# nogueira04/RaCFormer

Measured on AMD Instinct MI355X. Metric: samples/sec (6-cam 704x256, 900 queries, f8), higher is better.
Workload: dtype f32

## Files before the change

### include/racformer_hip.h

```cpp
#ifndef RACFORMER_HIP_H
#define RACFORMER_HIP_H

#include <stdint.h>

#ifdef __cplusplus
extern "C" {
#endif

#define RAC_ABI_VERSION 8
#define RAC_MAX_LEVELS 8
#define RAC_MAX_POINTS 128

enum { RAC_F32 = 0, RAC_BF16 = 1, RAC_I16 = 2  };

enum {
    RAC_E_ARG = -1,
    RAC_E_UNSUPPORTED = -2,
};

enum {
    RAC_OUT_SQCP = 0,
    RAC_OUT_BQGTPC = 1
};

int rac_abi_version(void);
const char *rac_last_error(void);

int rac_msmv_fwd(const void *const *feats, const int32_t *hw, int L, const float *loc,
                 const float *w, float *out, int S, int N, int Q, int P, int C, int dtype,
                 int out_layout, int T, int G, void *stream);

int rac_msda_fwd(const void *value, const int64_t *shapes, const int64_t *starts, const float *loc,
                 const float *attn, float *out, int bs, int keys, int heads, int dim, int Q, int L,
                 int P, int dtype, void *stream);

int rac_regroup_fwd(const float *in, void *out, int B, int T, int N, int G, int C, int H, int W,
                    int out_dtype, void *stream);

int rac_regroup_multi_fwd(int L, const float *const *ins, void *const *outs, const int32_t *hw, int B, int T, int N, int G,
                          int C, int out_dtype, void *stream);

int rac_box_prep_fwd(const float *query_bbox, float *table, int num_boxes, const float *pc_range, void *stream);

int rac_sampling4d_fwd(const void *const *feats, const int32_t *hw, int L, const float *query_bbox,
                       const float *box_table, const float *offsets, const float *ray_logits, const float *scale_logits,
                       const float *time_diff, const float *lidar2img, float *out, float *loc_out,
                       float *w_out, const unsigned char *view_in, int ld_off, int ld_ray, int ld_scale, int B, int T, int N,
                       int G, int Q,
                       int NP, int D, int C, const float *pc_range, const float *depth_base, float d_region,
                       float image_h, float image_w, float eps, int dtype, int compact, void *stream);

int rac_bev_sampling_fwd(const void *value, const float *query_bbox, const float *box_table, const float *offsets,
                         const float *ray_logits, const float *scale_logits, const float *queue_logits,
                         const float *time_diff, float *out, float *loc_out, int ld_off, int ld_ray,
                         int ld_scale, int ld_queue, int B, int T, int Q, int heads, int NP, int D, int H, int W,
                         int dim, const float *pc_range, const float *depth_base, float d_region, int dtype,
                         void *stream);

int rac_bev_sampling_multi_fwd(int nstreams, const void *const *values, const float *const *offsets,
                               const float *const *ray_logits, const float *const *scale_logits,
                               const float *const *queue_logits, float *const *outs, const float *query_bbox,
                               const float *box_table, const float *time_diff, int ld_off, int ld_ray, int ld_scale,
                               int ld_queue, int B, int T, int Q, int heads, int NP, int D, int H, int W, int dim,
                               const float *pc_range, const float *depth_base, float d_region, int dtype, void *stream);

int rac_quant_i16_fwd(const float *values, void *q, float *scale, int64_t blocks, void *stream);

int rac_bev_sampling_multi_q16_fwd(int nstreams, const void *const *values, const float *const *value_scales,
                                   const float *const *offsets, const float *const *ray_logits,
                                   const float *const *scale_logits, const float *const *queue_logits, float *const *outs,
                                   const float *query_bbox, const float *box_table, const float *time_diff, int ld_off,
                                   int ld_ray, int ld_scale, int ld_queue, int B, int T, int Q, int heads, int NP, int D,
                                   int H, int W, int dim, const float *pc_range, const float *depth_base, float d_region,
                                   void *stream);

int rac_sasa_fwd(const float *qkv, const float *tau, const float *query_bbox, const float *box_table, float *out,
                 int ld_qkv, int ld_tau, int B, int Q, int heads, int dim, const float *pc_range, void *stream);

enum {
    RAC_SPLIT_KCAT = 0,
    RAC_SPLIT_LINES = 1
};

int rac_add_ln_fwd(const float *a, int num_partials, int64_t partial_stride, int ld_a, float a_scale, const float *residual,
                   const float *bias, const float *gamma, const float *beta, const float *post_residual,
                   float *out, int ld_out, int rows, int dim, float eps, int relu, void *split_out,
                   float split_scale, int split_pad, int split_layout, void *stream);

int rac_head_finish_fwd(float *cls, int64_t n_cls, const float *xy, float *box, int64_t rows, int code_size,
                        const float *pc_range, void *stream);

int rac_pe_head_fwd(const float *x, int ld_x, const float *weight, const float *bias, const float *gamma,
                    const float *beta, float *out, int rows, int dim, float eps, void *stream);

int rac_refine_fwd(const float *proposal, const float *delta, const float *time_diff_safe, float *bbox_pred,
                   float *bbox_xy, int B, int Q, int T, float num_ray, void *stream);

int rac_layer_boundary_fwd(const float *proposal, const float *delta, const float *time_diff_safe, float *bbox_pred,
                           float *bbox_xy, float *box_table, const float *pc_range, const float *pe_weight,
                           const float *pe_bias, const float *pe_gamma, const float *pe_beta, float *pe_out, int B, int Q,
                           int T, int dim, float num_ray, float eps, void *stream);

enum {
    RAC_MIX_F32 = 0,
    RAC_MIX_F16X3 = 1
};

int rac_mixing_fwd(const float *x, const float *params, float param_scale, float *out, void *out_split,
                   float split_scale, int ld_params, int num_query, int groups, int in_points, int channels, int out_points,
                   float eps, int mfma_mode, void *stream);

int rac_mixing_sampled_fwd(const void *const *feats, const int32_t *hw, int L, const float *query_bbox, const float *box_table,
                           const float *offsets, const float *ray_logits, const float *scale_logits, const float *time_diff,
                           const float *lidar2img, float *loc_out, float *w_out, const unsigned char *view_in, int ld_off,
                           int ld_ray, int ld_scale, int B, int T, int N, int G, int Q, int NP, int D, int C,
                           const float *pc_range, const float *depth_base, float d_region, float image_h, float image_w,
                           float eps_proj, int dtype, const float *params, float param_scale, float *out, void *out_split,
                           float split_scale, int ld_params, int out_points, float eps_ln, void *stream);

int rac_gemm_split_pack_fwd(const float *weight, void *image, int N, int K, float scale, void *stream);

int rac_outproj_fwd(const void *z_image, const void *w_image, float *partials, int M, int N, int K, int slices, void *stream);

int rac_generator_fwd(const void *x_image, const void *w_image, const float *bias, float alpha, float *out, int64_t ld_out, int M,
                      int N, int K, void *stream);

int rac_value_proj_fwd(const float *x, const void *w_image, float w_alpha, const float *add, const float *bias, float *out,
                       int frames, int channels, int HW, int features, void *stream);
int rac_value_proj_q16_fwd(const float *x, const void *w_image, float w_alpha, const float *add, const float *bias, void *q,
                           float *scale, int frames, int channels, int HW, int features, void *stream);

int rac_absmax_fwd(const float *const *srcs, const int64_t *counts, int num, float floor_value, float *amax_out,
                   void *stream);
int rac_conv_pack_fwd(const float *src, const float *amax, void *xs, int N, int C, int H, int W, int c_total,
                      int c_offset, void *stream);
int rac_conv_pack_bias_fwd(const float *src, const float *bias, const float *amax, void *xs, int N, int C, int H, int W,
                           int c_total, int c_offset, int frames_per_group, int live_per_group, void *stream);
int rac_conv3x3_fwd(const void *xs, const void *ws, const float *bias, const float *pixel_bias, const float *amax,
                    float w_alpha, float *out, int N, int H, int W, int Cin, int Cout, void *stream);
int rac_conv3x3_q16_fwd(const void *xs, const void *ws, const float *bias, const float *pixel_bias, const float *amax,
                        float w_alpha, void *q, float *scale, int N, int H, int W, int Cin, int Cout, void *stream);

int rac_fpn_conv_fwd(const void *xs, const void *ws, const float *bias, const float *amax, float w_alpha, float *out,
                     int num_images, int H, int W, int Cin, int num_cams, void *stream);

int rac_gru_gate_fwd(const float *gates, const float *h_prev, int64_t h_prev_bstride, float *h_out, int64_t h_out_bstride,
                     const float *bias_map, float *h_out2, int64_t h_out2_bstride, int B, int C, int HW, void *stream);
int rac_upsample2x_fwd(const float *src, float *dst, int64_t planes, int h, int w, void *stream);

#define RAC_ROWGEMM_MAX_BATCH 3
typedef struct {
    const float *a;
    int64_t partial_stride;
    const float *bias0, *residual, *gamma, *beta, *post;
    float *x_out;
    void *split_out;
    int ld_a, num_partials, ld_res, ld_post, ld_xout, relu, split_pad, split_layout;
    float a_scale, eps, split_scale;
} rac_rowseg;
typedef struct {
    rac_rowseg seg[3];
    const float *w, *b;
    float *out;
    int num_seg, N, ld_out, relu_from;
} rac_rowgemm;
int rac_rowgemm_fwd(const rac_rowgemm *descs, int num, int rows, void *stream);

int rac_conv3x3s2_fwd(const void *xs, const void *ws, const float *bias, const float *amax, float w_alpha, float *out,
                      int out_channels_total, int N, int H, int W, int Cin, int Cin_image, int Cout, void *stream);

int rac_decode_fwd(const float *cls_scores, const float *bbox_preds, float *out, int num_query, int num_classes,
                   int max_num, const float *post_center_range, float score_threshold, int use_threshold, void *stream);

int rac_msmv_bwd(const float *grad_out, const void *const *feats, const int32_t *hw, int L, const float *loc,
                 const float *w, void *const *grad_feats, float *grad_loc, float *grad_w, int S, int N, int Q,
                 int P, int C, void *stream);
int rac_msda_bwd(const float *grad_out, const float *value, const int64_t *shapes, const int64_t *starts,
                 const float *loc, const float *attn, float *grad_value, float *grad_loc, float *grad_attn,
                 int bs, int keys, int heads, int dim, int Q, int L, int P, void *stream);

int rac_bev_pool_v2_fwd(const float *depth, const float *feat, float *out, const int32_t *ranks_depth,
                        const int32_t *ranks_feat, const int32_t *ranks_bev, const int32_t *interval_lengths,
                        const int32_t *interval_starts, int c, int n_intervals, void *stream);
int rac_bev_pool_v2_bwd(const float *out_grad, float *depth_grad, float *feat_grad, const float *depth,
                        const float *feat, const int32_t *ranks_depth, const int32_t *ranks_feat,
                        const int32_t *ranks_bev, const int32_t *interval_lengths, const int32_t *interval_starts,
                        int c, int n_intervals, void *stream);

enum { RAC_CD_IMAGE = 0, RAC_CD_F32 = 1, RAC_CD_GRU = 2 };
typedef struct {
    const float *amax;
    float mul, add;
} rac_cd_scale;
typedef struct {
    int live, stride, first;
} rac_cd_frames;
typedef struct {
    int mode, conv_stride;
    int N, H, W;
    const void *in_img;
    int in_chunks_total, in_chunk0, chunks;
    rac_cd_frames in_frames;
    rac_cd_scale in_scale;
    const void *ws;
    float w_alpha;
    int Cout;
    const float *bias;
    void *out_img;
    int out_chunks_total, out_chunk0;
    rac_cd_frames out_frames;
    rac_cd_scale out_scale;
    float *out_f32;
    const float *pixel_map;
    const float *xpart;
    rac_cd_frames xpart_frames;
    const float *h_prev;
    rac_cd_frames h_prev_frames;
    float *h_out;
    rac_cd_frames h_out_frames;
} rac_conv_direct;
int rac_conv_direct_fwd(const rac_conv_direct *desc, void *stream);

int rac_upsample2x_image_fwd(const float *src, void *img, int frames, int h, int w, int C, float bound, void *stream);

int rac_conv3x3_temporal_fwd(const void *xs, const void *ws, const float *pixel_bias_live, const float *pixel_bias_dead,
                             const float *amax, float w_alpha, float *out, void *q, float *scale, int N, int H, int W, int Cin,
                             int Cin_dead, int frames_per_group, int live_per_group, void *stream);

#ifdef __cplusplus
}
#endif
#endif
```

### racformer_amd/_lib.py

```python
import ctypes
import os

import torch

_HERE = os.path.dirname(os.path.abspath(__file__))
LIB_PATH = os.environ.get("RACFORMER_HIP_LIB") or os.path.join(_HERE, "csrc", "libracformer_hip.so")
RAC_F32, RAC_BF16, RAC_I16 = 0, 1, 2
OUT_SQCP, OUT_BQGTPC = 0, 1
MIX_F32, MIX_F16X3 = 0, 1
_lib = None

_vp, _i, _f = ctypes.c_void_p, ctypes.c_int, ctypes.c_float
SIGNATURES = {
    "rac_abi_version": (_i, []),
    "rac_last_error": (ctypes.c_char_p, []),
    "rac_msmv_fwd": (_i, [_vp, _vp, _i, _vp, _vp, _vp, _i, _i, _i, _i, _i, _i, _i, _i, _i, _vp]),
    "rac_msda_fwd": (_i, [_vp, _vp, _vp, _vp, _vp, _vp, _i, _i, _i, _i, _i, _i, _i, _i, _vp]),
    "rac_regroup_fwd": (_i, [_vp, _vp, _i, _i, _i, _i, _i, _i, _i, _i, _vp]),
    "rac_regroup_multi_fwd": (_i, [_i, _vp, _vp, _vp, _i, _i, _i, _i, _i, _i, _vp]),
    "rac_box_prep_fwd": (_i, [_vp, _vp, _i, _vp, _vp]),
    "rac_sampling4d_fwd": (_i, [_vp, _vp, _i] + [_vp] * 11 + [_i] * 3 + [_i] * 8 + [_vp, _vp] + [_f] * 4 + [_i, _i, _vp]),
    "rac_msmv_bwd": (_i, [_vp, _vp, _vp, _i, _vp, _vp, _vp, _vp, _vp] + [_i] * 5 + [_vp]),
    "rac_msda_bwd": (_i, [_vp] * 9 + [_i] * 7 + [_vp]),
    "rac_bev_pool_v2_fwd": (_i, [_vp] * 8 + [_i, _i, _vp]),
    "rac_bev_pool_v2_bwd": (_i, [_vp] * 10 + [_i, _i, _vp]),
    "rac_add_ln_fwd": (_i, [_vp, _i, ctypes.c_int64, _i, _f] + [_vp] * 6 + [_i, _i, _i, _f, _i, _vp, _f, _i, _i, _vp]),
    "rac_pe_head_fwd": (_i, [_vp, _i] + [_vp] * 5 + [_i, _i, _f, _vp]),
    "rac_layer_boundary_fwd": (_i, [_vp] * 12 + [_i] * 4 + [_f, _f, _vp]),
    "rac_refine_fwd": (_i, [_vp] * 5 + [_i] * 3 + [_f, _vp]),
    "rac_head_finish_fwd": (_i, [_vp, ctypes.c_int64, _vp, _vp, ctypes.c_int64, _i, _vp, _vp]),
    "rac_mixing_fwd": (_i, [_vp, _vp, _f, _vp, _vp, _f] + [_i] * 6 + [_f, _i, _vp]),
    "rac_mixing_sampled_fwd": (_i, [_vp, _vp, _i] + [_vp] * 10 + [_i] * 3 + [_i] * 8 + [_vp, _vp] + [_f] * 4 + [_i]
                               + [_vp, _f, _vp, _vp, _f, _i, _i, _f, _vp]),
    "rac_sasa_fwd": (_i, [_vp] * 5 + [_i] * 6 + [_vp, _vp]),
    "rac_decode_fwd": (_i, [_vp, _vp, _vp, _i, _i, _i, _vp, _f, _i, _vp]),
    "rac_rowgemm_fwd": (_i, [_vp, _i, _i, _vp]),
    "rac_gemm_split_pack_fwd": (_i, [_vp, _vp, _i, _i, _f, _vp]),
    "rac_value_proj_fwd": (_i, [_vp, _vp, _f, _vp, _vp, _vp, _i, _i, _i, _i, _vp]),
    "rac_value_proj_q16_fwd": (_i, [_vp, _vp, _f, _vp, _vp, _vp, _vp, _i, _i, _i, _i, _vp]),
    "rac_outproj_fwd": (_i, [_vp, _vp, _vp, _i, _i, _i, _i, _vp]),
    "rac_generator_fwd": (_i, [_vp, _vp, _vp, _f, _vp, ctypes.c_int64, _i, _i, _i, _vp]),
    "rac_gru_gate_fwd": (_i, [_vp, _vp, ctypes.c_int64, _vp, ctypes.c_int64, _vp, _vp, ctypes.c_int64, _i, _i, _i, _vp]),
    "rac_upsample2x_fwd": (_i, [_vp, _vp, ctypes.c_int64, _i, _i, _vp]),
    "rac_absmax_fwd": (_i, [_vp, _vp, _i, _f, _vp, _vp]),
    "rac_conv_pack_fwd": (_i, [_vp, _vp, _vp] + [_i] * 6 + [_vp]),
    "rac_conv_pack_bias_fwd": (_i, [_vp, _vp, _vp, _vp] + [_i] * 8 + [_vp]),
    "rac_conv3x3_fwd": (_i, [_vp] * 5 + [_f, _vp] + [_i] * 5 + [_vp]),
    "rac_conv3x3_q16_fwd": (_i, [_vp] * 5 + [_f, _vp, _vp] + [_i] * 5 + [_vp]),
    "rac_fpn_conv_fwd": (_i, [_vp] * 4 + [_f, _vp] + [_i] * 5 + [_vp]),
    "rac_conv3x3s2_fwd": (_i, [_vp] * 4 + [_f, _vp] + [_i] * 7 + [_vp]),
    "rac_bev_sampling_fwd": (_i, [_vp] * 10 + [_i] * 4 + [_i] * 9 + [_vp, _vp, _f, _i, _vp]),
    "rac_bev_sampling_multi_fwd": (_i, [_i] + [_vp] * 9 + [_i] * 4 + [_i] * 9 + [_vp, _vp, _f, _i, _vp]),
    "rac_bev_sampling_multi_q16_fwd": (_i, [_i] + [_vp] * 10 + [_i] * 4 + [_i] * 9 + [_vp, _vp, _f, _vp]),
    "rac_quant_i16_fwd": (_i, [_vp, _vp, _vp, ctypes.c_int64, _vp]),
    "rac_conv_direct_fwd": (_i, [_vp, _vp]),
    "rac_upsample2x_image_fwd": (_i, [_vp, _vp, _i, _i, _i, _i, _f, _vp]),
    "rac_conv3x3_temporal_fwd": (_i, [_vp, _vp, _vp, _vp, _vp, _f, _vp, _vp, _vp] + [_i] * 7 + [_vp]),
}


class RowSeg(ctypes.Structure):
    _fields_ = [("a", _vp), ("partial_stride", ctypes.c_int64), ("bias0", _vp), ("residual", _vp), ("gamma", _vp),
                ("beta", _vp), ("post", _vp), ("x_out", _vp), ("split_out", _vp), ("ld_a", _i), ("num_partials", _i),
                ("ld_res", _i), ("ld_post", _i), ("ld_xout", _i), ("relu", _i), ("split_pad", _i), ("split_layout", _i), ("a_scale", _f),
                ("eps", _f), ("split_scale", _f)]


class RowGemm(ctypes.Structure):
    _fields_ = [("seg", RowSeg * 3), ("w", _vp), ("b", _vp), ("out", _vp), ("num_seg", _i), ("N", _i), ("ld_out", _i),
                ("relu_from", _i)]


class CdScale(ctypes.Structure):
    _fields_ = [("amax", _vp), ("mul", _f), ("add", _f)]


class CdFrames(ctypes.Structure):
    _fields_ = [("live", _i), ("stride", _i), ("first", _i)]


class ConvDirect(ctypes.Structure):
    _fields_ = [("mode", _i), ("conv_stride", _i), ("N", _i), ("H", _i), ("W", _i), ("in_img", _vp), ("in_chunks_total", _i),
                ("in_chunk0", _i), ("chunks", _i), ("in_frames", CdFrames), ("in_scale", CdScale), ("ws", _vp), ("w_alpha", _f),
                ("Cout", _i), ("bias", _vp), ("out_img", _vp), ("out_chunks_total", _i), ("out_chunk0", _i),
                ("out_frames", CdFrames), ("out_scale", CdScale), ("out_f32", _vp), ("pixel_map", _vp), ("xpart", _vp),
                ("xpart_frames", CdFrames), ("h_prev", _vp), ("h_prev_frames", CdFrames), ("h_out", _vp),
                ("h_out_frames", CdFrames)]


CD_IMAGE, CD_F32, CD_GRU = 0, 1, 2


def lib():
    global _lib
    if _lib is None:
        if not os.path.exists(LIB_PATH):
            raise RuntimeError(
                f"racformer_amd: HIP library not built ({LIB_PATH}); run "
                "`python -c 'import __graft_entry__ as g; g.build()'` or `make -C racformer_amd/csrc`. "
                "There is no CPU fallback for the hot path.")
        handle = ctypes.CDLL(LIB_PATH)
        for name, (res, args) in SIGNATURES.items():
            fn = getattr(handle, name)
            fn.restype, fn.argtypes = res, args
        _lib = handle
    return _lib


def check(rc, what):
    if rc != 0:
        msg = lib().rac_last_error().decode(errors="replace")
        raise RuntimeError(f"{what} failed (rc={rc}): {msg}")


def stream_ptr():
    try:
        return ctypes.c_void_p(torch._C._cuda_getCurrentRawStream(torch._C._cuda_getDevice()))
    except AttributeError:
        return ctypes.c_void_p(torch.cuda.current_stream().cuda_stream)


def dtype_code(t):
    if t.dtype == torch.float32:
        return RAC_F32
    if t.dtype == torch.bfloat16:
        return RAC_BF16
    raise TypeError(f"racformer_amd: unsupported feature dtype {t.dtype} (float32 or bfloat16)")


def require_gpu(*tensors, what="op"):
    for t in tensors:
        if not t.is_cuda:
            raise RuntimeError(f"racformer_amd.{what}: tensor must be a CUDA tensor "
                               "(HIP device); the hot path has no CPU fallback")
        if not t.is_contiguous():
            raise RuntimeError(f"racformer_amd.{what}: tensor has to be contiguous")


def ptr(t):
    return ctypes.c_void_p(t.data_ptr())


class KernelTimer:

    def __init__(self, only=None):
        self.events = {}
        self.only = set(only) if only is not None else None

    def record(self, name):
        if self.only is not None and name not in self.only:
            return None
        start, end = torch.cuda.Event(enable_timing=True), torch.cuda.Event(enable_timing=True)
        self.events.setdefault(name, []).append((start, end))
        return start, end

    def mean_ms(self, name):
        ev = self.events.get(name, [])
        if not ev:
            return None
        return sum(s.elapsed_time(e) for s, e in ev) / len(ev)

    def reset(self):
        self.events = {}


timer = None
```

### racformer_amd/csrc/add_ln.hip

```cpp
#include "rac_common.h"

#define ALN_MAX_V 4

__device__ __forceinline__ float aln_wave_sum(float v)
{
#pragma unroll
    for (int off = 32; off >= 1; off >>= 1)
        v += __shfl_xor(v, off, 64);
    return v;
}

__global__ __launch_bounds__(256) void add_ln_kernel(const float *__restrict__ a, int S, long pstride, int ld_a, float a_scale,
                                                     const float *__restrict__ residual, const float *__restrict__ bias,
                                                     const float *__restrict__ gamma, const float *__restrict__ beta,
                                                     const float *__restrict__ post, float *__restrict__ out, int ld_out,
                                                     int rows, int dim, float eps, int relu,
                                                     _Float16 *__restrict__ split_out, float split_scale, int split_pad, int split_lines)
{
    const int row = blockIdx.x * 4 + (threadIdx.x >> 6);
    const int lane = threadIdx.x & 63;
    if (row >= rows)
        return;
    const int nv = dim >> 2;
    rac_f4 x[ALN_MAX_V];
    float sum = 0.f;
#pragma unroll
    for (int k = 0; k < ALN_MAX_V; ++k) {
        const int c = lane + 64 * k;
        x[k] = (rac_f4){0.f, 0.f, 0.f, 0.f};
        if (c < nv) {
            rac_f4 v = rac_ld4(a + (size_t)row * ld_a + c * 4);
            for (int s0 = 1; s0 < S; s0 += 8) {
                rac_f4 w[8];
#pragma unroll
                for (int j = 0; j < 8; ++j) {
                    w[j] = (rac_f4){0.f, 0.f, 0.f, 0.f};
                    if (s0 + j < S)
                        w[j] = rac_ld4(a + (size_t)(s0 + j) * pstride + (size_t)row * ld_a + c * 4);
                }
#pragma unroll
                for (int j = 0; j < 8; ++j) {
                    v.x += w[j].x; v.y += w[j].y; v.z += w[j].z; v.w += w[j].w;
                }
            }
            v.x *= a_scale; v.y *= a_scale; v.z *= a_scale; v.w *= a_scale;
            if (bias) {
                const rac_f4 w = rac_ld4(bias + c * 4);
                v.x += w.x; v.y += w.y; v.z += w.z; v.w += w.w;
            }
            if (residual) {
                const rac_f4 w = rac_ld4(residual + (size_t)row * dim + c * 4);
                v.x += w.x; v.y += w.y; v.z += w.z; v.w += w.w;
            }
            x[k] = v;
            sum += (v.x + v.y) + (v.z + v.w);
        }
    }
    const float mean = aln_wave_sum(sum) / (float)dim;
    float sq = 0.f;
#pragma unroll
    for (int k = 0; k < ALN_MAX_V; ++k)
        if (lane + 64 * k < nv) {
            const float d0 = x[k].x - mean, d1 = x[k].y - mean, d2 = x[k].z - mean, d3 = x[k].w - mean;
            sq += (d0 * d0 + d1 * d1) + (d2 * d2 + d3 * d3);
        }
    const float rstd = 1.f / sqrtf(aln_wave_sum(sq) / (float)dim + eps);
#pragma unroll
    for (int k = 0; k < ALN_MAX_V; ++k) {
        const int c = lane + 64 * k;
        if (c < nv) {
            const rac_f4 g = rac_ld4(gamma + c * 4), b = rac_ld4(beta + c * 4);
            rac_f4 y;
            y.x = (x[k].x - mean) * rstd * g.x + b.x;
            y.y = (x[k].y - mean) * rstd * g.y + b.y;
            y.z = (x[k].z - mean) * rstd * g.z + b.z;
            y.w = (x[k].w - mean) * rstd * g.w + b.w;
            if (relu) {
                y.x = fmaxf(y.x, 0.f); y.y = fmaxf(y.y, 0.f); y.z = fmaxf(y.z, 0.f); y.w = fmaxf(y.w, 0.f);
            }
            if (post) {
                const rac_f4 w = rac_ld4(post + (size_t)row * dim + c * 4);
                y.x += w.x; y.y += w.y; y.z += w.z; y.w += w.w;
            }
            *reinterpret_cast<rac_f4 *>(out + (size_t)row * ld_out + c * 4) = y;
            if (split_out) {
                rac_h4 hi, lo;
                rac_split_f16(y.x * split_scale, hi.x, lo.x);
                rac_split_f16(y.y * split_scale, hi.y, lo.y);
                rac_split_f16(y.z * split_scale, hi.z, lo.z);
                rac_split_f16(y.w * split_scale, hi.w, lo.w);
                if (split_lines) {
                    _Float16 *dl = split_out + (size_t)row * (2 * dim) + (c >> 3) * 64 + (c & 7) * 4;
                    *reinterpret_cast<rac_h4 *>(dl) = hi;
                    *reinterpret_cast<rac_h4 *>(dl + 32) = lo;
                    continue;
                }
                _Float16 *dst = split_out + (size_t)row * (3 * dim + split_pad) + c * 4;
                *reinterpret_cast<rac_h4 *>(dst) = hi;
                *reinterpret_cast<rac_h4 *>(dst + dim) = hi;
                *reinterpret_cast<rac_h4 *>(dst + 2 * dim) = lo;
                if (split_pad && c == 0) {
                    _Float16 *pad = split_out + (size_t)row * (3 * dim + split_pad) + 3 * dim;
                    for (int i = 0; i < split_pad; ++i)
                        pad[i] = i < 2 ? (_Float16)split_scale : (_Float16)0.f;
                }
            }
        }
    }
}

__global__ __launch_bounds__(256) void add_ln_many_kernel(const float *__restrict__ a, int S, long pstride, int ld_a, float a_scale,
                                                          const float *__restrict__ residual, const float *__restrict__ bias,
                                                          const float *__restrict__ gamma, const float *__restrict__ beta,
                                                          const float *__restrict__ post, float *__restrict__ out, int ld_out,
                                                          int rows, float eps, int relu,
                                                          _Float16 *__restrict__ split_out, float split_scale, int split_pad, int split_lines)
{
    __shared__ rac_f4 part[3][64];
    const int row = blockIdx.x, wave = threadIdx.x >> 6, lane = threadIdx.x & 63;
    const int per = (S + 3) / 4, s_lo = wave * per, s_hi = min(S, s_lo + per);
    rac_f4 v = {0.f, 0.f, 0.f, 0.f};
    for (int s0 = s_lo; s0 < s_hi; s0 += 8) {
        rac_f4 w[8];
#pragma unroll
        for (int j = 0; j < 8; ++j) {
            w[j] = (rac_f4){0.f, 0.f, 0.f, 0.f};
            if (s0 + j < s_hi)
                w[j] = rac_ld4(a + (size_t)(s0 + j) * pstride + (size_t)row * ld_a + lane * 4);
        }
#pragma unroll
        for (int j = 0; j < 8; ++j) {
            v.x += w[j].x; v.y += w[j].y; v.z += w[j].z; v.w += w[j].w;
        }
    }
    if (wave > 0)
        part[wave - 1][lane] = v;
    __syncthreads();
    if (wave > 0)
        return;
#pragma unroll
    for (int k = 0; k < 3; ++k) {
        const rac_f4 w = part[k][lane];
        v.x += w.x; v.y += w.y; v.z += w.z; v.w += w.w;
    }
    v.x *= a_scale; v.y *= a_scale; v.z *= a_scale; v.w *= a_scale;
    if (bias) {
        const rac_f4 w = rac_ld4(bias + lane * 4);
        v.x += w.x; v.y += w.y; v.z += w.z; v.w += w.w;
    }
    if (residual) {
        const rac_f4 w = rac_ld4(residual + (size_t)row * 256 + lane * 4);
        v.x += w.x; v.y += w.y; v.z += w.z; v.w += w.w;
    }
    const float mean = aln_wave_sum((v.x + v.y) + (v.z + v.w)) / 256.f;
    const float d0 = v.x - mean, d1 = v.y - mean, d2 = v.z - mean, d3 = v.w - mean;
    const float rstd = 1.f / sqrtf(aln_wave_sum((d0 * d0 + d1 * d1) + (d2 * d2 + d3 * d3)) / 256.f + eps);
    const rac_f4 g = rac_ld4(gamma + lane * 4), b = rac_ld4(beta + lane * 4);
    rac_f4 y = {d0 * rstd * g.x + b.x, d1 * rstd * g.y + b.y, d2 * rstd * g.z + b.z, d3 * rstd * g.w + b.w};
    if (relu) {
        y.x = fmaxf(y.x, 0.f); y.y = fmaxf(y.y, 0.f); y.z = fmaxf(y.z, 0.f); y.w = fmaxf(y.w, 0.f);
    }
    if (post) {
        const rac_f4 w = rac_ld4(post + (size_t)row * 256 + lane * 4);
        y.x += w.x; y.y += w.y; y.z += w.z; y.w += w.w;
    }
    *reinterpret_cast<rac_f4 *>(out + (size_t)row * ld_out + lane * 4) = y;
    if (split_out) {
        rac_h4 hi, lo;
        rac_split_f16(y.x * split_scale, hi.x, lo.x);
        rac_split_f16(y.y * split_scale, hi.y, lo.y);
        rac_split_f16(y.z * split_scale, hi.z, lo.z);
        rac_split_f16(y.w * split_scale, hi.w, lo.w);
        if (split_lines) {
            _Float16 *dl = split_out + (size_t)row * 512 + (lane >> 3) * 64 + (lane & 7) * 4;
            *reinterpret_cast<rac_h4 *>(dl) = hi;
            *reinterpret_cast<rac_h4 *>(dl + 32) = lo;
        } else {
            _Float16 *dst = split_out + (size_t)row * (768 + split_pad) + lane * 4;
            *reinterpret_cast<rac_h4 *>(dst) = hi;
            *reinterpret_cast<rac_h4 *>(dst + 256) = hi;
            *reinterpret_cast<rac_h4 *>(dst + 512) = lo;
            if (split_pad && lane == 0) {
                _Float16 *pad = split_out + (size_t)row * (768 + split_pad) + 768;
                for (int i = 0; i < split_pad; ++i)
                    pad[i] = i < 2 ? (_Float16)split_scale : (_Float16)0.f;
            }
        }
    }
}

__global__ __launch_bounds__(256) void pe_head_kernel(const float *__restrict__ x, int ld_x, const float *__restrict__ W,
                                                      const float *__restrict__ bias, const float *__restrict__ gamma,
                                                      const float *__restrict__ beta, float *__restrict__ out, int rows, float eps)
{
    const int row = blockIdx.x * 4 + (threadIdx.x >> 6);
    const int lane = threadIdx.x & 63;
    if (row >= rows)
        return;
    const float x0 = x[(size_t)row * ld_x], x1 = x[(size_t)row * ld_x + 1], x2 = x[(size_t)row * ld_x + 2];
    float v[4];
#pragma unroll
    for (int j = 0; j < 4; ++j) {
        const int c = lane * 4 + j;
        v[j] = W[c * 3] * x0 + W[c * 3 + 1] * x1 + W[c * 3 + 2] * x2 + bias[c];
    }
    const float mean = aln_wave_sum((v[0] + v[1]) + (v[2] + v[3])) / 256.f;
    const float d0 = v[0] - mean, d1 = v[1] - mean, d2 = v[2] - mean, d3 = v[3] - mean;
    const float rstd = 1.f / sqrtf(aln_wave_sum((d0 * d0 + d1 * d1) + (d2 * d2 + d3 * d3)) / 256.f + eps);
    const rac_f4 g = rac_ld4(gamma + lane * 4), b = rac_ld4(beta + lane * 4);
    rac_f4 y = {fmaxf(d0 * rstd * g.x + b.x, 0.f), fmaxf(d1 * rstd * g.y + b.y, 0.f), fmaxf(d2 * rstd * g.z + b.z, 0.f),
                fmaxf(d3 * rstd * g.w + b.w, 0.f)};
    *reinterpret_cast<rac_f4 *>(out + (size_t)row * 256 + lane * 4) = y;
}

extern "C" int rac_add_ln_fwd(const float *a, int num_partials, int64_t partial_stride, int ld_a, float a_scale, const float *residual,
                              const float *bias, const float *gamma, const float *beta, const float *post_residual,
                              float *out, int ld_out, int rows, int dim, float eps, int relu, void *split_out,
                              float split_scale, int split_pad, int split_layout, void *stream)
{
    RAC_CHECK_ARG(split_layout == RAC_SPLIT_KCAT || (split_layout == RAC_SPLIT_LINES && dim % 32 == 0 && split_pad == 0),
                  "rac_add_ln_fwd: split_layout=%d (RAC_SPLIT_LINES needs dim %% 32 == 0 and split_pad == 0)", split_layout);
    RAC_CHECK_ARG(rows >= 0 && dim >= 4 && dim % 4 == 0 && dim <= 256 * ALN_MAX_V, "rac_add_ln_fwd: dim=%d (multiple of 4, <= %d)", dim, 256 * ALN_MAX_V);
    RAC_CHECK_ARG(num_partials >= 1, "rac_add_ln_fwd: num_partials=%d", num_partials);
    RAC_CHECK_ARG(!split_out || split_pad == 0 || (split_pad >= 2 && split_pad % 4 == 0), "rac_add_ln_fwd: split_pad=%d (0, or a multiple of 4)", split_pad);
    RAC_CHECK_ARG(ld_a >= dim && ld_out >= dim && ld_a % 4 == 0 && ld_out % 4 == 0, "rac_add_ln_fwd: row strides ld_a=%d ld_out=%d", ld_a, ld_out);
    if (rows == 0)
        return 0;
    RAC_CHECK_ARG(a && gamma && beta && out, "rac_add_ln_fwd: null pointer");
    if (dim == 256 && num_partials >= 8) {
        hipLaunchKernelGGL(add_ln_many_kernel, dim3(rows), dim3(256), 0, (hipStream_t)stream, a, num_partials, (long)partial_stride, ld_a,
                           a_scale, residual, bias, gamma, beta, post_residual, out, ld_out, rows, eps, relu,
                           reinterpret_cast<_Float16 *>(split_out), split_scale, split_pad, split_layout == RAC_SPLIT_LINES ? 1 : 0);
        return rac_launch_status("rac_add_ln_fwd");
    }
    hipLaunchKernelGGL(add_ln_kernel, dim3((rows + 3) / 4), dim3(256), 0, (hipStream_t)stream, a, num_partials,
                       (long)partial_stride, ld_a, a_scale, residual, bias, gamma, beta, post_residual, out, ld_out, rows, dim, eps, relu,
                       reinterpret_cast<_Float16 *>(split_out), split_scale, split_pad, split_layout == RAC_SPLIT_LINES ? 1 : 0);
    return rac_launch_status("rac_add_ln_fwd");
}

extern "C" int rac_pe_head_fwd(const float *x, int ld_x, const float *weight, const float *bias, const float *gamma,
                               const float *beta, float *out, int rows, int dim, float eps, void *stream)
{
    RAC_CHECK_ARG(dim == 256 && rows >= 0 && ld_x >= 3, "rac_pe_head_fwd: dim=%d (built for 256), ld_x=%d", dim, ld_x);
    if (rows == 0)
        return 0;
    RAC_CHECK_ARG(x && weight && bias && gamma && beta && out, "rac_pe_head_fwd: null pointer");
    hipLaunchKernelGGL(pe_head_kernel, dim3((rows + 3) / 4), dim3(256), 0, (hipStream_t)stream, x, ld_x, weight, bias, gamma,
                       beta, out, rows, eps);
    return rac_launch_status("rac_pe_head_fwd");
}
```

### racformer_amd/csrc/rac_common.h

```cpp
#pragma once
#include <hip/hip_runtime.h>
#include <stdint.h>
#include <stdio.h>
#include "../../include/racformer_hip.h"

#define RAC_WAVE 64

void rac_set_error(const char *fmt, ...);

int rac_set_dynamic_lds_once(int id, const void *func, int bytes);
enum { RAC_ATTR_GEMM_SPLIT = 0, RAC_ATTR_GENERATOR, RAC_ATTR_CONV3X3, RAC_ATTR_CONV3X3S2, RAC_ATTR_MIXING_F32, RAC_ATTR_MIXING_F16,
       RAC_ATTR_VALUE_PROJ, RAC_ATTR_FPN_CONV, RAC_ATTR_GENERATOR4, RAC_ATTR_CONV3X3_Q16, RAC_ATTR_VALUE_PROJ_Q16, RAC_ATTR_MIXING_SAMPLED,
       RAC_ATTR_CD_GRU, RAC_ATTR_CD_S2_8, RAC_ATTR_CD_S2_2, RAC_ATTR_CD_S2_3, RAC_ATTR_CD_IMG_2, RAC_ATTR_CD_F32_1, RAC_ATTR_CD_F32_2,
       RAC_ATTR_CD_F32_4, RAC_ATTR_VALUE_PROJ_BIAS, RAC_ATTR_VALUE_PROJ_Q16_BIAS };

template <int I>
struct rac_ic {
    static constexpr int value = I;
};
template <int B, int E, typename F>
__device__ __forceinline__ void rac_static_for(F &&f)
{
    if constexpr (B < E) {
        f(rac_ic<B>{});
        rac_static_for<B + 1, E>(f);
    }
}

#define RAC_CHECK_ARG(cond, ...)            \
    do {                                    \
        if (!(cond)) {                      \
            rac_set_error(__VA_ARGS__);     \
            return RAC_E_ARG;               \
        }                                   \
    } while (0)

static inline int rac_launch_status(const char *what)
{
    hipError_t e = hipGetLastError();
    if (e != hipSuccess) {
        rac_set_error("%s: %s", what, hipGetErrorString(e));
        return (int)e;
    }
    return 0;
}

__device__ __forceinline__ float rac_bf16_to_f32(unsigned short v)
{
    return __uint_as_float(((unsigned)v) << 16);
}

struct alignas(16) rac_f4 {
    float x, y, z, w;
};

__device__ __forceinline__ rac_f4 rac_ld4(const float *p)
{
    return *reinterpret_cast<const rac_f4 *>(p);
}
#ifndef RAC_STREAM_NT
#define RAC_STREAM_NT 1
#endif
typedef float rac_f4v __attribute__((ext_vector_type(4)));
__device__ __forceinline__ rac_f4 rac_ld4_stream(const float *p)
{
#if RAC_STREAM_NT
    const rac_f4v v = __builtin_nontemporal_load(reinterpret_cast<const rac_f4v *>(p));
    return rac_f4{v.x, v.y, v.z, v.w};
#else
    return rac_ld4(p);
#endif
}
__device__ __forceinline__ void rac_st4_stream(float *p, const rac_f4 v)
{
#if RAC_STREAM_NT
    __builtin_nontemporal_store((rac_f4v){v.x, v.y, v.z, v.w}, reinterpret_cast<rac_f4v *>(p));
#else
    *reinterpret_cast<rac_f4 *>(p) = v;
#endif
}
__device__ __forceinline__ rac_f4 rac_ld4(const unsigned short *p)
{
    uint2 r = *reinterpret_cast<const uint2 *>(p);
    rac_f4 o;
    o.x = __uint_as_float(r.x << 16);
    o.y = __uint_as_float(r.x & 0xffff0000u);
    o.z = __uint_as_float(r.y << 16);
    o.w = __uint_as_float(r.y & 0xffff0000u);
    return o;
}

#ifndef RAC_GATHER_PACKED_FMA
#define RAC_GATHER_PACKED_FMA 0
#endif
#if RAC_GATHER_PACKED_FMA && !defined(RAC_DIAGNOSTIC_BUILD)
#error "RAC_GATHER_PACKED_FMA is a diagnostic switch (DESIGN 3.12): packed FP32 accumulation goes wrong beside another stream's MFMA kernels"
#endif
typedef float rac_f2v __attribute__((ext_vector_type(2)));
struct rac_acc4 {
#if RAC_GATHER_PACKED_FMA
    rac_f2v a01, a23;
#else
    float a0, a1, a2, a3;
#endif
};
__device__ __forceinline__ rac_acc4 rac_acc4_zero()
{
#if RAC_GATHER_PACKED_FMA
    return rac_acc4{(rac_f2v){0.f, 0.f}, (rac_f2v){0.f, 0.f}};
#else
    return rac_acc4{0.f, 0.f, 0.f, 0.f};
#endif
}
__device__ __forceinline__ void rac_tap_fma(rac_acc4 &acc, float x, float y, float z, float w4, float w)
{
#if RAC_GATHER_PACKED_FMA
    const rac_f2v w2 = {w, w};
    acc.a01 = __builtin_elementwise_fma((rac_f2v){x, y}, w2, acc.a01);
    acc.a23 = __builtin_elementwise_fma((rac_f2v){z, w4}, w2, acc.a23);
#else
    acc.a0 = __builtin_fmaf(x, w, acc.a0);
    acc.a1 = __builtin_fmaf(y, w, acc.a1);
    acc.a2 = __builtin_fmaf(z, w, acc.a2);
    acc.a3 = __builtin_fmaf(w4, w, acc.a3);
    asm volatile("" : "+v"(acc.a0), "+v"(acc.a1), "+v"(acc.a2), "+v"(acc.a3));
#endif
}
__device__ __forceinline__ void rac_acc4_get(const rac_acc4 &acc, float &x, float &y, float &z, float &w)
{
#if RAC_GATHER_PACKED_FMA
    x = acc.a01.x; y = acc.a01.y; z = acc.a23.x; w = acc.a23.y;
#else
    x = acc.a0; y = acc.a1; z = acc.a2; w = acc.a3;
#endif
}

struct alignas(8) rac_h4 {
    _Float16 x, y, z, w;
};

__device__ __forceinline__ void rac_split_f16(float v, _Float16 &hi, _Float16 &lo)
{
    hi = (_Float16)v;
    lo = (_Float16)(v - (float)hi);
}

__device__ __forceinline__ float rac_act_scale(float amax)
{
    if (!(amax > 1.0e-30f) || !(amax < 3.0e38f))
        return 1.f;
    const int ex = (int)((__float_as_uint(amax) >> 23) & 0xffu) - 126;
    return __uint_as_float((unsigned)(14 - ex + 127) << 23);
}

__device__ __forceinline__ unsigned rac_absbits(float x) { return __float_as_uint(x) & 0x7fffffffu; }
__device__ __forceinline__ unsigned rac_absbits4(float x, float y, float z, float w)
{
    return max(max(rac_absbits(x), rac_absbits(y)), max(rac_absbits(z), rac_absbits(w)));
}
__device__ __forceinline__ void rac_q16_factors(unsigned block_max_bits, float &up, float &dn)
{
    int eb = (int)((block_max_bits >> 23) & 255u);
    if (eb == 255) {
        up = 0.f;
        dn = __uint_as_float(0x7fc00000u);
        return;
    }
    eb = eb < 15 ? 15 : eb;
    up = __uint_as_float((unsigned)(268 - eb) << 23);
    dn = __uint_as_float((unsigned)(eb - 14) << 23);
}
__device__ __forceinline__ int rac_q16(float x, float up)
{
    return (int)fminf(fmaxf(rintf(x * up), -32767.f), 32767.f);
}
__device__ __forceinline__ uint2 rac_q16x4(float x, float y, float z, float w, float up)
{
    uint2 o;
    o.x = ((unsigned)rac_q16(x, up) & 0xffffu) | ((unsigned)rac_q16(y, up) << 16);
    o.y = ((unsigned)rac_q16(z, up) & 0xffffu) | ((unsigned)rac_q16(w, up) << 16);
    return o;
}

#if defined(RAC_CLOCK_STAMPS) && defined(RAC_DIAGNOSTIC_BUILD)
#define RAC_CLOCK_WGS 1024
#define RAC_CLOCK_DECL(name) __device__ unsigned long long name##_clock_buf[RAC_CLOCK_WGS * 4];
#define RAC_CLOCK_BEGIN() const unsigned long long clk_t0_ = __builtin_amdgcn_s_memtime(), clk_r0_ = __builtin_amdgcn_s_memrealtime()
#define RAC_CLOCK_END(name, wg)                                                  \
    do {                                                                         \
        if ((threadIdx.x & 63) == 0 && threadIdx.x < 64 && (wg) < RAC_CLOCK_WGS) { \
            name##_clock_buf[(wg) * 4 + 0] = clk_t0_;                            \
            name##_clock_buf[(wg) * 4 + 1] = clk_r0_;                            \
            name##_clock_buf[(wg) * 4 + 2] = __builtin_amdgcn_s_memtime();       \
            name##_clock_buf[(wg) * 4 + 3] = __builtin_amdgcn_s_memrealtime();   \
        }                                                                        \
    } while (0)
#define RAC_CLOCK_READER(name)                                                                                           \
    extern "C" int rac_dbg_clock_##name(unsigned long long *host_out, int n_wgs)                                         \
    {                                                                                                                    \
        if (n_wgs > RAC_CLOCK_WGS)                                                                                       \
            n_wgs = RAC_CLOCK_WGS;                                                                                       \
        hipDeviceSynchronize();                                                                                          \
        return (int)hipMemcpyFromSymbol(host_out, HIP_SYMBOL(name##_clock_buf), sizeof(unsigned long long) * 4 * n_wgs, 0, \
                                        hipMemcpyDeviceToHost);                                                          \
    }
#else
#define RAC_CLOCK_DECL(name)
#define RAC_CLOCK_BEGIN()
#define RAC_CLOCK_END(name, wg)
#define RAC_CLOCK_READER(name)
#endif
```

### racformer_amd/csrc/refine.hip

```cpp
#include "rac_common.h"

#define REF_TWO_PI 6.283185307179586f

__device__ __forceinline__ float ref_sigmoid(float x) { return 1.f / (1.f + expf(-x)); }

__device__ __forceinline__ float ref_inverse_sigmoid(float x)
{
    x = fminf(fmaxf(x, 0.f), 1.f);
    const float x1 = fmaxf(x, 1e-5f), x2 = fmaxf(1.f - x, 1e-5f);
    return logf(x1 / x2);
}

__global__ __launch_bounds__(256) void refine_kernel(const float *__restrict__ prop, const float *__restrict__ delta,
                                                     const float *__restrict__ td_safe, float *__restrict__ pred,
                                                     float *__restrict__ xy, int n, int Q, int T, float num_ray)
{
    const int i = blockIdx.x * 256 + threadIdx.x;
    if (i >= n)
        return;
    const float *p = prop + (size_t)i * 10, *d = delta + (size_t)i * 10;
    float o[10];
    o[0] = p[0] + (ref_sigmoid(d[0]) * 2.f - 1.f) / num_ray;
    o[1] = ref_sigmoid(d[1] + ref_inverse_sigmoid(p[1]));
    o[2] = ref_sigmoid(d[2] + ref_inverse_sigmoid(p[2]));
#pragma unroll
    for (int k = 3; k < 10; ++k)
        o[k] = d[k];
    if (T > 1) {
        const float td = td_safe[(i / Q) * T + 1];
        o[8] = o[8] / td;
        o[9] = o[9] / td;
    }
    float *pp = pred + (size_t)i * 10, *px = xy + (size_t)i * 10;
#pragma unroll
    for (int k = 0; k < 10; ++k)
        pp[k] = o[k];
    const float ang = o[0] * REF_TWO_PI, rad = o[1] * 65.0f;
    px[0] = fminf(fmaxf((51.2f + rad * cosf(ang)) / 102.4f, 0.f), 1.f);
    px[1] = fminf(fmaxf((51.2f + rad * sinf(ang)) / 102.4f, 0.f), 1.f);
#pragma unroll
    for (int k = 2; k < 10; ++k)
        px[k] = o[k];
}

extern "C" int rac_refine_fwd(const float *proposal, const float *delta, const float *time_diff_safe, float *bbox_pred,
                              float *bbox_xy, int B, int Q, int T, float num_ray, void *stream)
{
    RAC_CHECK_ARG(B >= 0 && Q >= 0 && T >= 1 && num_ray > 0.f, "rac_refine_fwd: bad sizes B=%d Q=%d T=%d", B, Q, T);
    if (B * Q == 0)
        return 0;
    RAC_CHECK_ARG(proposal && delta && time_diff_safe && bbox_pred && bbox_xy, "rac_refine_fwd: null pointer");
    const int n = B * Q;
    hipLaunchKernelGGL(refine_kernel, dim3((n + 255) / 256), dim3(256), 0, (hipStream_t)stream, proposal, delta,
                       time_diff_safe, bbox_pred, bbox_xy, n, Q, T, num_ray);
    return rac_launch_status("rac_refine_fwd");
}

__device__ __forceinline__ float hf_nan_to_num(float v)
{
    if (v != v)
        return 0.f;
    return fminf(fmaxf(v, -3.4028234663852886e38f), 3.4028234663852886e38f);
}

__global__ __launch_bounds__(256) void head_finish_kernel(float *__restrict__ cls, long n_cls, const float *__restrict__ xy,
                                                          float *__restrict__ box, long rows, float x0, float y0, float z0,
                                                          float sx, float sy, float sz)
{
    const long i = (long)blockIdx.x * 256 + threadIdx.x;
    if (i < n_cls)
        cls[i] = hf_nan_to_num(cls[i]);
    if (i < rows) {
#pragma clang fp contract(off)
        const float *s = xy + i * 10;
        float v[10];
#pragma unroll
        for (int k = 0; k < 10; ++k)
            v[k] = hf_nan_to_num(s[k]);
        float *d = box + i * 10;
        d[0] = v[0] * sx + x0; d[1] = v[1] * sy + y0; d[2] = v[3]; d[3] = v[4]; d[4] = v[2] * sz + z0;
        d[5] = v[5]; d[6] = v[6]; d[7] = v[7]; d[8] = v[8]; d[9] = v[9];
    }
}

extern "C" int rac_head_finish_fwd(float *cls, int64_t n_cls, const float *xy, float *box, int64_t rows, int code_size,
                                   const float *pc_range, void *stream)
{
    RAC_CHECK_ARG(n_cls >= 0 && rows >= 0 && code_size == 10, "rac_head_finish_fwd: n_cls=%lld rows=%lld code_size=%d (10)",
                  (long long)n_cls, (long long)rows, code_size);
    const long n = n_cls > rows ? n_cls : rows;
    if (n == 0)
        return 0;
    RAC_CHECK_ARG((cls || n_cls == 0) && (rows == 0 || (xy && box)) && pc_range && xy != box, "rac_head_finish_fwd: null pointer or xy aliases box");
    hipLaunchKernelGGL(head_finish_kernel, dim3((unsigned)((n + 255) / 256)), dim3(256), 0, (hipStream_t)stream, cls, (long)n_cls, xy, box,
                       (long)rows, pc_range[0], pc_range[1], pc_range[2], pc_range[3] - pc_range[0], pc_range[4] - pc_range[1],
                       pc_range[5] - pc_range[2]);
    return rac_launch_status("rac_head_finish_fwd");
}

__device__ __forceinline__ float lb_wave_sum(float v)
{
#pragma unroll
    for (int off = 32; off >= 1; off >>= 1)
        v += __shfl_xor(v, off, 64);
    return v;
}

__global__ __launch_bounds__(256) void layer_boundary_kernel(const float *__restrict__ prop, const float *__restrict__ delta,
                                                             const float *__restrict__ td_safe, float *__restrict__ pred,
                                                             float *__restrict__ xy, float *__restrict__ table,
                                                             const float *__restrict__ W, const float *__restrict__ bias,
                                                             const float *__restrict__ gamma, const float *__restrict__ beta,
                                                             float *__restrict__ h_out, int n, int Q, int T, float num_ray,
                                                             float eps, float p0, float p1, float p2, float sx, float sy, float sz)
{
    const int i = blockIdx.x * 4 + (threadIdx.x >> 6);
    const int lane = threadIdx.x & 63;
    if (i >= n)
        return;
    const float *p = prop + (size_t)i * 10, *d = delta + (size_t)i * 10;
    float o[10];
    o[0] = p[0] + (ref_sigmoid(d[0]) * 2.f - 1.f) / num_ray;
    o[1] = ref_sigmoid(d[1] + ref_inverse_sigmoid(p[1]));
    o[2] = ref_sigmoid(d[2] + ref_inverse_sigmoid(p[2]));
#pragma unroll
    for (int k = 3; k < 10; ++k)
        o[k] = d[k];
    if (T > 1) {
        const float td = td_safe[(i / Q) * T + 1];
        o[8] = o[8] / td;
        o[9] = o[9] / td;
    }
    const float ang = o[0] * REF_TWO_PI, rad = o[1] * 65.0f;
    const float xn = fminf(fmaxf((51.2f + rad * cosf(ang)) / 102.4f, 0.f), 1.f);
    const float yn = fminf(fmaxf((51.2f + rad * sinf(ang)) / 102.4f, 0.f), 1.f);
    if (lane == 0) {
        float *pp = pred + (size_t)i * 10, *px = xy + (size_t)i * 10, *t = table + (size_t)i * 8;
#pragma unroll
        for (int k = 0; k < 10; ++k)
            pp[k] = o[k];
        px[0] = xn;
        px[1] = yn;
#pragma unroll
        for (int k = 2; k < 10; ++k)
            px[k] = o[k];
        const float yaw = atan2f(o[6], o[7]);
        t[0] = xn * sx + p0;
        t[1] = yn * sy + p1;
        t[2] = o[2] * sz + p2;
        t[3] = expf(o[3]);
        t[4] = expf(o[4]);
        t[5] = expf(o[5]);
        t[6] = cosf(yaw);
        t[7] = sinf(yaw);
    }
    float v[4];
#pragma unroll
    for (int j = 0; j < 4; ++j) {
        const int c = lane * 4 + j;
        v[j] = W[c * 3] * o[0] + W[c * 3 + 1] * o[1] + W[c * 3 + 2] * o[2] + bias[c];
    }
    const float mean = lb_wave_sum((v[0] + v[1]) + (v[2] + v[3])) / 256.f;
    const float d0 = v[0] - mean, d1 = v[1] - mean, d2 = v[2] - mean, d3 = v[3] - mean;
    const float rstd = 1.f / sqrtf(lb_wave_sum((d0 * d0 + d1 * d1) + (d2 * d2 + d3 * d3)) / 256.f + eps);
    const rac_f4 g = rac_ld4(gamma + lane * 4), b = rac_ld4(beta + lane * 4);
    rac_f4 y = {fmaxf(d0 * rstd * g.x + b.x, 0.f), fmaxf(d1 * rstd * g.y + b.y, 0.f), fmaxf(d2 * rstd * g.z + b.z, 0.f),
                fmaxf(d3 * rstd * g.w + b.w, 0.f)};
    *reinterpret_cast<rac_f4 *>(h_out + (size_t)i * 256 + lane * 4) = y;
}

extern "C" int rac_layer_boundary_fwd(const float *proposal, const float *delta, const float *time_diff_safe, float *bbox_pred,
                                      float *bbox_xy, float *box_table, const float *pc_range, const float *pe_weight,
                                      const float *pe_bias, const float *pe_gamma, const float *pe_beta, float *pe_out, int B,
                                      int Q, int T, int dim, float num_ray, float eps, void *stream)
{
    RAC_CHECK_ARG(B >= 0 && Q >= 0 && T >= 1 && num_ray > 0.f && dim == 256, "rac_layer_boundary_fwd: bad sizes B=%d Q=%d T=%d dim=%d", B, Q, T, dim);
    if (B * Q == 0)
        return 0;
    RAC_CHECK_ARG(proposal && delta && time_diff_safe && bbox_pred && bbox_xy && box_table && pc_range && pe_weight && pe_bias &&
                      pe_gamma && pe_beta && pe_out,
                  "rac_layer_boundary_fwd: null pointer");
    const int n = B * Q;
    hipLaunchKernelGGL(layer_boundary_kernel, dim3((n + 3) / 4), dim3(256), 0, (hipStream_t)stream, proposal, delta,
                       time_diff_safe, bbox_pred, bbox_xy, box_table, pe_weight, pe_bias, pe_gamma, pe_beta, pe_out, n, Q, T,
                       num_ray, eps, pc_range[0], pc_range[1], pc_range[2], pc_range[3] - pc_range[0], pc_range[4] - pc_range[1],
                       pc_range[5] - pc_range[2]);
    return rac_launch_status("rac_layer_boundary_fwd");
}
```

### racformer_amd/csrc/rowgemm.hip

```cpp
#include "rac_common.h"

typedef float rg_f4 __attribute__((ext_vector_type(4)));

struct RowGemmArgs {
    rac_rowgemm d[RAC_ROWGEMM_MAX_BATCH];
    int rows;
};

__device__ __forceinline__ float rg_wave_sum(float v)
{
#pragma unroll
    for (int off = 32; off >= 1; off >>= 1)
        v += __shfl_xor(v, off, 64);
    return v;
}

template <int NSEG, int MT, bool EARLY>
__device__ __forceinline__ void rowgemm_body(const rac_rowgemm &d, int rows, float *sX)
{
    constexpr int K = 256 * NSEG, LD = K + 4, R = 16 * MT;
    const int tid = threadIdx.x, wave = tid >> 6, lane = tid & 63;
    const int row0 = blockIdx.x * R, n0 = blockIdx.y * 64;
    const bool first_slice = blockIdx.y == 0;
    const int li = lane & 15, lk = lane >> 4;
    const int col = n0 + 16 * wave + li;
    const int wrow = col < d.N ? col : d.N - 1;
    const float *bp = d.w + (size_t)wrow * K + 4 * lk;
    const int rot = (blockIdx.x * 5) & 15;
    rac_f4 bcur[16], bnxt[16];
    if (EARLY) {
#pragma unroll
        for (int u = 0; u < 16; ++u)
            bcur[u] = rac_ld4(bp + 16 * ((u + rot) & 15));
    }

#pragma unroll
    for (int s = 0; s < NSEG; ++s) {
        const rac_rowseg &g = d.seg[s];
        rac_f4 gm = {1.f, 1.f, 1.f, 1.f}, bt = {0.f, 0.f, 0.f, 0.f}, b0 = {0.f, 0.f, 0.f, 0.f};
        if (g.gamma) {
            gm = rac_ld4(g.gamma + lane * 4);
            bt = rac_ld4(g.beta + lane * 4);
        }
        if (g.bias0)
            b0 = rac_ld4(g.bias0 + lane * 4);
#pragma unroll 1
        for (int rb = 0; rb < MT; ++rb) {
            const int rbase = (wave * MT + rb) * 4;
            rac_f4 vv[4], rs[4];
#pragma unroll
            for (int rr = 0; rr < 4; ++rr) {
                const int row = row0 + rbase + rr;
                vv[rr] = (rac_f4){0.f, 0.f, 0.f, 0.f};
                rs[rr] = (rac_f4){0.f, 0.f, 0.f, 0.f};
                if (row < rows) {
                    vv[rr] = rac_ld4(g.a + (size_t)row * g.ld_a + lane * 4);
                    if (g.residual)
                        rs[rr] = rac_ld4(g.residual + (size_t)row * g.ld_res + lane * 4);
                }
            }
            for (int p = 1; p < g.num_partials; p += 2) {
                rac_f4 w[2][4];
#pragma unroll
                for (int j = 0; j < 2; ++j)
#pragma unroll
                    for (int rr = 0; rr < 4; ++rr) {
                        const int row = row0 + rbase + rr;
                        w[j][rr] = (rac_f4){0.f, 0.f, 0.f, 0.f};
                        if (row < rows && p + j < g.num_partials)
                            w[j][rr] = rac_ld4(g.a + (size_t)(p + j) * g.partial_stride + (size_t)row * g.ld_a + lane * 4);
                    }
#pragma unroll
                for (int rr = 0; rr < 4; ++rr) {
                    vv[rr].x += w[0][rr].x + w[1][rr].x; vv[rr].y += w[0][rr].y + w[1][rr].y;
                    vv[rr].z += w[0][rr].z + w[1][rr].z; vv[rr].w += w[0][rr].w + w[1][rr].w;
                }
            }
#pragma unroll
            for (int rr = 0; rr < 4; ++rr) {
                const int r = rbase + rr, row = row0 + r;
                rac_f4 v = vv[rr];
                if (row < rows) {
                    v.x = v.x * g.a_scale + b0.x + rs[rr].x; v.y = v.y * g.a_scale + b0.y + rs[rr].y;
                    v.z = v.z * g.a_scale + b0.z + rs[rr].z; v.w = v.w * g.a_scale + b0.w + rs[rr].w;
                }
                if (g.gamma) {
                    const float mean = rg_wave_sum((v.x + v.y) + (v.z + v.w)) / 256.f;
                    const float d0 = v.x - mean, d1 = v.y - mean, d2 = v.z - mean, d3 = v.w - mean;
                    const float rstd = 1.f / sqrtf(rg_wave_sum((d0 * d0 + d1 * d1) + (d2 * d2 + d3 * d3)) / 256.f + g.eps);
                    v.x = d0 * rstd * gm.x + bt.x; v.y = d1 * rstd * gm.y + bt.y;
                    v.z = d2 * rstd * gm.z + bt.z; v.w = d3 * rstd * gm.w + bt.w;
                }
                if (g.relu) {
                    v.x = fmaxf(v.x, 0.f); v.y = fmaxf(v.y, 0.f); v.z = fmaxf(v.z, 0.f); v.w = fmaxf(v.w, 0.f);
                }
                if (g.post && row < rows) {
                    const rac_f4 w = rac_ld4(g.post + (size_t)row * g.ld_post + lane * 4);
                    v.x += w.x; v.y += w.y; v.z += w.z; v.w += w.w;
                }
                *reinterpret_cast<rac_f4 *>(sX + r * LD + 256 * s + lane * 4) = v;
                if (first_slice && row < rows) {
                    if (g.x_out)
                        *reinterpret_cast<rac_f4 *>(g.x_out + (size_t)row * g.ld_xout + lane * 4) = v;
                    if (g.split_out) {
                        rac_h4 hi, lo;
                        rac_split_f16(v.x * g.split_scale, hi.x, lo.x);
                        rac_split_f16(v.y * g.split_scale, hi.y, lo.y);
                        rac_split_f16(v.z * g.split_scale, hi.z, lo.z);
                        rac_split_f16(v.w * g.split_scale, hi.w, lo.w);
                        if (g.split_layout == RAC_SPLIT_LINES) {
                            _Float16 *dst = reinterpret_cast<_Float16 *>(g.split_out) + (size_t)row * 512 + (lane >> 3) * 64 + (lane & 7) * 4;
                            *reinterpret_cast<rac_h4 *>(dst) = hi;
                            *reinterpret_cast<rac_h4 *>(dst + 32) = lo;
                        } else {
                            _Float16 *dst = reinterpret_cast<_Float16 *>(g.split_out) + (size_t)row * (768 + g.split_pad);
                            *reinterpret_cast<rac_h4 *>(dst + lane * 4) = hi;
                            *reinterpret_cast<rac_h4 *>(dst + 256 + lane * 4) = hi;
                            *reinterpret_cast<rac_h4 *>(dst + 512 + lane * 4) = lo;
                            if (lane < g.split_pad)
                                dst[768 + lane] = lane < 2 ? (_Float16)g.split_scale : (_Float16)0.f;
                        }
                    }
                }
            }
        }
    }
    __syncthreads();

    const float *ap = sX + li * LD + 4 * lk;
    if (!EARLY) {
#pragma unroll
        for (int u = 0; u < 16; ++u)
            bcur[u] = rac_ld4(bp + 16 * ((u + rot) & 15));
    }
    rg_f4 acc[MT][2];
#pragma unroll
    for (int m = 0; m < MT; ++m)
        acc[m][0] = acc[m][1] = (rg_f4){0.f, 0.f, 0.f, 0.f};
#pragma unroll
    for (int sgm = 0; sgm < NSEG; ++sgm) {
        if (sgm + 1 < NSEG) {
#pragma unroll
            for (int u = 0; u < 16; ++u)
                bnxt[u] = rac_ld4(bp + 256 * (sgm + 1) + 16 * ((u + rot) & 15));
        }
#pragma unroll
        for (int u = 0; u < 16; ++u) {
            const int ko = 256 * sgm + 16 * ((u + rot) & 15);
#pragma unroll
            for (int m = 0; m < MT; ++m) {
                const rac_f4 a4 = *reinterpret_cast<const rac_f4 *>(ap + 16 * m * LD + ko);
                acc[m][0] = __builtin_amdgcn_mfma_f32_16x16x4f32(a4.x, bcur[u].x, acc[m][0], 0, 0, 0);
                acc[m][1] = __builtin_amdgcn_mfma_f32_16x16x4f32(a4.y, bcur[u].y, acc[m][1], 0, 0, 0);
                acc[m][0] = __builtin_amdgcn_mfma_f32_16x16x4f32(a4.z, bcur[u].z, acc[m][0], 0, 0, 0);
                acc[m][1] = __builtin_amdgcn_mfma_f32_16x16x4f32(a4.w, bcur[u].w, acc[m][1], 0, 0, 0);
            }
        }
        if (sgm + 1 < NSEG) {
#pragma unroll
            for (int u = 0; u < 16; ++u)
                bcur[u] = bnxt[u];
        }
    }
    const float bv = d.b ? d.b[wrow] : 0.f;
    const bool relu = col >= d.relu_from;
#pragma unroll
    for (int m = 0; m < MT; ++m)
#pragma unroll
        for (int r = 0; r < 4; ++r) {
            const int row = row0 + 16 * m + 4 * lk + r;
            float v = (acc[m][0][r] + acc[m][1][r]) + bv;
            if (relu)
                v = fmaxf(v, 0.f);
            if (row < rows && col < d.N)
                d.out[(size_t)row * d.ld_out + col] = v;
        }
}

template <int NSEG, int MT, bool EARLY>
__global__ __launch_bounds__(256, EARLY ? 2 : 4) void rowgemm_kernel(const RowGemmArgs a)
{
    extern __shared__ float smem[];
    const rac_rowgemm &d = a.d[blockIdx.z];
    if ((int)blockIdx.y * 64 >= d.N)
        return;
    rowgemm_body<NSEG, MT, EARLY>(d, a.rows, smem);
}

extern "C" int rac_rowgemm_fwd(const rac_rowgemm *descs, int num, int rows, void *stream)
{
    RAC_CHECK_ARG(descs && num >= 1 && num <= RAC_ROWGEMM_MAX_BATCH && rows >= 0, "rac_rowgemm_fwd: num=%d rows=%d", num, rows);
    if (rows == 0)
        return 0;
    RowGemmArgs a;
    int max_n = 0, max_seg = 0;
    for (int i = 0; i < num; ++i) {
        const rac_rowgemm &d = descs[i];
        RAC_CHECK_ARG(d.num_seg >= 1 && d.num_seg <= 3 && d.N >= 1 && d.w && d.out && d.ld_out >= d.N,
                      "rac_rowgemm_fwd: GEMM %d: num_seg=%d N=%d ld_out=%d", i, d.num_seg, d.N, d.ld_out);
        for (int s = 0; s < d.num_seg; ++s) {
            const rac_rowseg &g = d.seg[s];
            RAC_CHECK_ARG(g.a && g.ld_a >= 256 && g.ld_a % 4 == 0 && g.num_partials >= 1 && g.partial_stride % 4 == 0,
                          "rac_rowgemm_fwd: GEMM %d segment %d: source rows (ld_a=%d, partials=%d)", i, s, g.ld_a, g.num_partials);
            RAC_CHECK_ARG((!g.gamma) == (!g.beta), "rac_rowgemm_fwd: GEMM %d segment %d: gamma / beta must come together", i, s);
            RAC_CHECK_ARG((!g.residual || g.ld_res % 4 == 0) && (!g.post || g.ld_post % 4 == 0) && (!g.x_out || g.ld_xout % 4 == 0),
                          "rac_rowgemm_fwd: GEMM %d segment %d: row strides must be multiples of 4", i, s);
            RAC_CHECK_ARG(!g.split_out || (g.split_pad >= 0 && g.split_pad <= 64 && g.split_pad % 4 == 0),
                          "rac_rowgemm_fwd: GEMM %d segment %d: split_pad=%d", i, s, g.split_pad);
        }
        RAC_CHECK_ARG(d.num_seg == descs[0].num_seg, "rac_rowgemm_fwd: batched GEMMs must have the same number of segments");
        a.d[i] = d;
        max_n = d.N > max_n ? d.N : max_n;
        max_seg = d.num_seg > max_seg ? d.num_seg : max_seg;
    }
    a.rows = rows;
    hipStream_t st = (hipStream_t)stream;
    const int R = 16;
    const size_t lds = (size_t)R * (256 * max_seg + 4) * sizeof(float);
    const dim3 grid((rows + R - 1) / R, (max_n + 63) / 64, num);
    if (max_seg == 1 && (long)grid.x * grid.y * grid.z > 512)
        hipLaunchKernelGGL((rowgemm_kernel<1, 1, false>), grid, dim3(256), lds, st, a);
    else if (max_seg == 1)
        hipLaunchKernelGGL((rowgemm_kernel<1, 1, true>), grid, dim3(256), lds, st, a);
    else if (max_seg == 2)
        hipLaunchKernelGGL((rowgemm_kernel<2, 1, true>), grid, dim3(256), lds, st, a);
    else
        hipLaunchKernelGGL((rowgemm_kernel<3, 1, true>), grid, dim3(256), lds, st, a);
    return rac_launch_status("rac_rowgemm_fwd");
}
```

### racformer_amd/fused.py

```python
import ctypes
import functools

import torch

from . import _lib


@functools.lru_cache(maxsize=64)
def _depth_base(d_region, depth_num):
    vals = torch.linspace(-d_region, d_region, depth_num).tolist()
    return (ctypes.c_float * depth_num)(*vals)


def _rows(t, width, what):
    if not t.is_cuda or t.dtype != torch.float32:
        raise RuntimeError(f"racformer_amd.{what}: expected a float32 CUDA tensor")
    if t.shape[-1] != width or t.stride(-1) != 1 or (t.dim() == 3 and t.shape[0] > 1 and t.stride(0) != t.shape[1] * t.stride(1)):
        raise RuntimeError(f"racformer_amd.{what}: expected [B,Q,{width}] rows with unit inner stride")
    return _lib.ptr(t), int(t.stride(-2))


def box_prep(query_bbox, pc_range):
    _lib.require_gpu(query_bbox, what="box_prep")
    table = torch.empty(query_bbox.shape[:-1] + (8,), device=query_bbox.device, dtype=torch.float32)
# ... 405 lines not shown
                                    _lib.ptr(norm.weight), _lib.ptr(norm.bias), _lib.ptr(out), rows, linear.weight.shape[0],
                                    float(norm.eps), _lib.stream_ptr())
    _lib.check(rc, "rac_pe_head_fwd")
    return out


def pack_conv3x3_weight(weight, cout=256):
    import math
    w = weight.detach().float()
    co, ci, kh, kw = w.shape
    amax = float(w.abs().max())
    if (kh, kw) != (3, 3) or co != cout or ci % 32 != 0 or not (amax > 0.0) or amax != amax or amax == float("inf"):
        return None, None
    s = 13 - math.frexp(amax)[1] + 1
    ws = (w * (2.0 ** s)).permute(2, 3, 1, 0).reshape(9, ci // 32, 32, co).permute(0, 1, 3, 2)
    hi = ws.to(torch.float16)
    lo = (ws - hi.float()).to(torch.float16)
    return torch.stack([hi, lo], dim=3).contiguous(), 2.0 ** (-s)


_conv_images = {}
_scratch_ns = [None]


class scratch_namespace:

    def __init__(self, key):
        self.key = key

    def __enter__(self):
        self.prev, _scratch_ns[0] = _scratch_ns[0], self.key
        return self

    def __exit__(self, *exc):
        _scratch_ns[0] = self.prev


def release_scratch(key):
    for k in [k for k in _conv_images if k[-1] == key]:
        del _conv_images[k]


class ConvImage:

    def __init__(self, N, H, W, cin, device):
        self.N, self.H, self.W, self.cin, self.dev = N, H, W, cin, device
        key = (N, H, W, cin, str(device), _scratch_ns[0])
        xs = _conv_images.get(key)
        if xs is None:
            xs = _conv_images[key] = torch.zeros(N, H + 2, W + 2, cin // 32, 2, 32, device=device, dtype=torch.float16)
        self.xs = xs
        self.amax = torch.empty(1, device=device, dtype=torch.float32)

    def begin(self, scan, floor=0.0):
        n = len(scan)
        _lib.require_gpu(*scan, what="ConvImage.begin")
        ptrs = (ctypes.c_void_p * max(n, 1))(*[t.data_ptr() for t in scan])
        counts = (ctypes.c_int64 * max(n, 1))(*[t.numel() for t in scan])
        _lib.check(_lib.lib().rac_absmax_fwd(ptrs, counts, n, float(floor), _lib.ptr(self.amax), _lib.stream_ptr()),
                   "rac_absmax_fwd")
        return self

    def pack(self, src, c_offset):
        _lib.require_gpu(src, what="ConvImage.pack")
        if tuple(src.shape[0:1] + src.shape[2:]) != (self.N, self.H, self.W) or src.dtype != torch.float32:
            raise RuntimeError("ConvImage.pack: sources must be float32 [N,C,H,W] matching the image")
        _lib.check(_lib.lib().rac_conv_pack_fwd(_lib.ptr(src), _lib.ptr(self.amax), _lib.ptr(self.xs), self.N, int(src.shape[1]),
                                                self.H, self.W, self.cin, int(c_offset), _lib.stream_ptr()), "rac_conv_pack_fwd")
        return self

    def pack_live(self, src, bias, c_offset, frames_per_group):
        _lib.require_gpu(src, what="ConvImage.pack_live")
        G = self.N // frames_per_group
        if self.N % frames_per_group != 0 or src.shape[0] % G != 0 or tuple(src.shape[2:]) != (self.H, self.W) or src.dtype != torch.float32:
            raise RuntimeError("ConvImage.pack_live: src must be float32 [groups * live, C, H, W] matching the image")
        _lib.check(_lib.lib().rac_conv_pack_bias_fwd(_lib.ptr(src), _lib.ptr(bias) if bias is not None else None, _lib.ptr(self.amax),
                                                     _lib.ptr(self.xs), self.N, int(src.shape[1]), self.H, self.W, self.cin, int(c_offset),
                                                     int(frames_per_group), int(src.shape[0] // G), _lib.stream_ptr()),
                   "rac_conv_pack_bias_fwd")
        return self

    def conv(self, ws, w_alpha, bias=None, pixel_bias=None, q16=False):
        N, H, W = self.N, self.H, self.W
        if pixel_bias is not None and (tuple(pixel_bias.shape) != (H * W, 256) or not pixel_bias.is_contiguous()
                                       or pixel_bias.dtype != torch.float32 or not pixel_bias.is_cuda):
            raise RuntimeError("ConvImage.conv: pixel_bias must be a contiguous float32 CUDA [H*W, 256] tensor")
        if q16:
            out = torch.empty(N, H * W, 4, 64, device=self.dev, dtype=torch.int16)
            scale = torch.empty(N, H * W, 4, device=self.dev, dtype=torch.float32)
        else:
            out = torch.empty(N, H, W, 256, device=self.dev, dtype=torch.float32)
        ev = _lib.timer.record("temporal_fusion_conv") if _lib.timer is not None else None
        if ev:
            ev[0].record()
        head = (_lib.ptr(self.xs), _lib.ptr(ws), _lib.ptr(bias) if bias is not None else None,
                _lib.ptr(pixel_bias) if pixel_bias is not None else None, _lib.ptr(self.amax), float(w_alpha))
        tail = (N, H, W, self.cin, 256, _lib.stream_ptr())
        if q16:
            rc, what = _lib.lib().rac_conv3x3_q16_fwd(*head, _lib.ptr(out), _lib.ptr(scale), *tail), "rac_conv3x3_q16_fwd"
        else:
            rc, what = _lib.lib().rac_conv3x3_fwd(*head, _lib.ptr(out), *tail), "rac_conv3x3_fwd"
        if ev:
            ev[1].record()
        _lib.check(rc, what)
        return (out, scale) if q16 else out

    def conv_temporal(self, ws, w_alpha, pixel_bias_live, pixel_bias_dead, cin_dead, frames_per_group, live_per_group, q16=False):
        N, H, W = self.N, self.H, self.W
        for pb in (pixel_bias_live, pixel_bias_dead):
            if tuple(pb.shape) != (H * W, 256) or not pb.is_contiguous() or pb.dtype != torch.float32 or not pb.is_cuda:
                raise RuntimeError("ConvImage.conv_temporal: the per-pixel maps must be contiguous float32 CUDA [H*W, 256] tensors")
        if q16:
            out = torch.empty(N, H * W, 4, 64, device=self.dev, dtype=torch.int16)
            scale = torch.empty(N, H * W, 4, device=self.dev, dtype=torch.float32)
        else:
            out, scale = torch.empty(N, H, W, 256, device=self.dev, dtype=torch.float32), None
        ev = _lib.timer.record("temporal_fusion_conv") if _lib.timer is not None else None
        if ev:
            ev[0].record()
        rc = _lib.lib().rac_conv3x3_temporal_fwd(_lib.ptr(self.xs), _lib.ptr(ws), _lib.ptr(pixel_bias_live), _lib.ptr(pixel_bias_dead),
                                                 _lib.ptr(self.amax), float(w_alpha), None if q16 else _lib.ptr(out),
                                                 _lib.ptr(out) if q16 else None, _lib.ptr(scale) if q16 else None, N, H, W, self.cin,
                                                 int(cin_dead), int(frames_per_group), int(live_per_group), _lib.stream_ptr())
        if ev:
            ev[1].record()
        _lib.check(rc, "rac_conv3x3_temporal_fwd")
        return (out, scale) if q16 else out

    def conv_s2(self, ws, w_alpha, bias, cin, out=None):
        N, H, W = self.N, self.H, self.W
        if out is None:
            out = torch.empty(N, 64, H // 2, W // 2, device=self.dev, dtype=torch.float32)
        elif not out.is_contiguous() or tuple(out.shape[0:1] + out.shape[2:]) != (N, H // 2, W // 2) or out.shape[1] < 64:
            raise RuntimeError("ConvImage.conv_s2: out must be a contiguous [N, >=64, H/2, W/2] tensor")
        _lib.check(_lib.lib().rac_conv3x3s2_fwd(_lib.ptr(self.xs), _lib.ptr(ws), _lib.ptr(bias) if bias is not None else None,
                                                _lib.ptr(self.amax), float(w_alpha), _lib.ptr(out), int(out.shape[1]), N, H, W,
                                                int(cin), self.cin, 64, _lib.stream_ptr()), "rac_conv3x3s2_fwd")
        return out


def conv3x3_fused(sources, ws, w_alpha, bias, bounds=None, pixel_bias=None):
    _lib.require_gpu(*sources, ws, what="conv3x3_fused")
    N, _, H, W = sources[0].shape
    cin = sum(int(t.shape[1]) for t in sources)
    bounds = list(bounds) if bounds is not None else [None] * len(sources)
    img = ConvImage(N, H, W, cin, sources[0].device)
    img.begin([t for t, bnd in zip(sources, bounds) if bnd is None], max([0.0] + [float(b) for b in bounds if b is not None]))
    off = 0
    for t in sources:
        img.pack(t, off)
        off += int(t.shape[1])
    return img.conv(ws, w_alpha, bias, pixel_bias)


def act_image(tag, frames, H, W, channels, device):
    key = ("act", tag, frames, H, W, channels, str(device), _scratch_ns[0])
    img = _conv_images.get(key)
    if img is None:
        img = _conv_images[key] = torch.zeros(frames, H + 2, W + 2, channels // 32, 2, 32, device=device, dtype=torch.float16)
    return img


def _cd_scale(amax=None, mul=0.0, add=0.0):
    return _lib.CdScale(_lib.ptr(amax) if amax is not None else None, float(mul), float(add))


def _cd_frames(live=1, stride=1, first=0):
    return _lib.CdFrames(int(live), int(stride), int(first))


def conv_direct(mode, N, H, W, in_img, in_chunks_total, chunks, ws, w_alpha, cout, in_scale, conv_stride=1, in_chunk0=0,
                in_frames=None, bias=None, out_img=None, out_chunks_total=0, out_chunk0=0, out_frames=None, out_scale=None,
                out_f32=None, pixel_map=None, xpart=None, xpart_frames=None, h_prev=None, h_prev_frames=None, h_out=None,
                h_out_frames=None):
    opt = lambda t: _lib.ptr(t) if t is not None else None
    fr = lambda f: _cd_frames(*(f or (1, 1, 0)))
    d = _lib.ConvDirect()
    d.mode, d.conv_stride, d.N, d.H, d.W = int(mode), int(conv_stride), int(N), int(H), int(W)
    d.in_img, d.in_chunks_total, d.in_chunk0, d.chunks = opt(in_img), int(in_chunks_total), int(in_chunk0), int(chunks)
    d.in_frames, d.in_scale = fr(in_frames), _cd_scale(*in_scale)
    d.ws, d.w_alpha, d.Cout, d.bias = opt(ws), float(w_alpha), int(cout), opt(bias)
    d.out_img, d.out_chunks_total, d.out_chunk0 = opt(out_img), int(out_chunks_total), int(out_chunk0)
    d.out_frames, d.out_scale = fr(out_frames), _cd_scale(*(out_scale or (None, 0.0, 0.0)))
    d.out_f32, d.pixel_map = opt(out_f32), opt(pixel_map)
    d.xpart, d.xpart_frames = opt(xpart), fr(xpart_frames)
    d.h_prev, d.h_prev_frames = opt(h_prev), fr(h_prev_frames)
    d.h_out, d.h_out_frames = opt(h_out), fr(h_out_frames)
    for t in (in_img, ws, bias, out_img, out_f32, pixel_map, xpart, h_prev, h_out):
        if t is not None:
            _lib.require_gpu(t, what="conv_direct")
    _lib.check(_lib.lib().rac_conv_direct_fwd(ctypes.byref(d), _lib.stream_ptr()), "rac_conv_direct_fwd")


def upsample2x_image(src, img, bound):
    _lib.require_gpu(src, img, what="upsample2x_image")
    frames, h, w, C = src.shape
    if tuple(img.shape) != (frames, 2 * h + 2, 2 * w + 2, C // 32, 2, 32) or img.dtype != torch.float16 or src.dtype != torch.float32:
        raise RuntimeError("upsample2x_image: src f32 [frames,h,w,C], img f16 [frames,2h+2,2w+2,C/32,2,32] expected")
    _lib.check(_lib.lib().rac_upsample2x_image_fwd(_lib.ptr(src), _lib.ptr(img), frames, h, w, C, float(bound), _lib.stream_ptr()),
               "rac_upsample2x_image_fwd")
    return img


def gru_gate_fused(gates, h_prev, h_out, bias_map=None, h_out2=None):
    B, C3, H, W = gates.shape
    C = C3 // 3
    if bias_map is not None and (tuple(bias_map.shape) != (C3, H, W) or not bias_map.is_contiguous() or not bias_map.is_cuda):
        raise RuntimeError("gru_gate_fused: bias_map must be a contiguous CUDA [3C,H,W] tensor")
    for t in (h_prev, h_out) + ((h_out2,) if h_out2 is not None else ()):
        if not t.is_cuda or tuple(t.shape) != (B, C, H, W) or t[0].is_contiguous() is False or t.dtype != torch.float32:
            raise RuntimeError("gru_gate_fused: h_prev / h_out must be float32 CUDA [B,C,H,W] views with contiguous batches")
    _lib.require_gpu(gates, what="gru_gate_fused")
    bs = lambda t: t.stride(0) if B > 1 else C * H * W
    rc = _lib.lib().rac_gru_gate_fwd(_lib.ptr(gates), _lib.ptr(h_prev), bs(h_prev), _lib.ptr(h_out), bs(h_out),
                                     _lib.ptr(bias_map) if bias_map is not None else None,
                                     _lib.ptr(h_out2) if h_out2 is not None else None, bs(h_out2) if h_out2 is not None else 0,
                                     B, C, H * W, _lib.stream_ptr())
    _lib.check(rc, "rac_gru_gate_fwd")
    return h_out


def upsample2x_fused(x):
    _lib.require_gpu(x, what="upsample2x_fused")
    N, C, h, w = x.shape
    out = torch.empty(N, C, 2 * h, 2 * w, device=x.device, dtype=torch.float32)
    rc = _lib.lib().rac_upsample2x_fwd(_lib.ptr(x), _lib.ptr(out), N * C, h, w, _lib.stream_ptr())
    _lib.check(rc, "rac_upsample2x_fwd")
    return out


def _rows2d(t, what):
    if not t.is_cuda or t.dtype != torch.float32 or t.stride(-1) != 1:
        raise RuntimeError(f"racformer_amd.rowgemm({what}): expected a float32 CUDA tensor with unit inner stride")
    if t.dim() == 3:
        if t.stride(0) != t.shape[1] * t.stride(1):
            raise RuntimeError(f"racformer_amd.rowgemm({what}): rows must be equally strided")
        ld = t.stride(1)
    elif t.dim() == 2:
        ld = t.stride(0)
    else:
        raise RuntimeError(f"racformer_amd.rowgemm({what}): expected [rows, W] or [B, Q, W]")
    return t, ctypes.c_void_p(t.data_ptr()), int(ld)


def row_seg(a, num_partials=1, a_scale=1.0, bias0=None, residual=None, norm=None, relu=False, post=None, x_out=None,
            split_out=None, split_lines=False):
    g = _lib.RowSeg()
    keep = []
    if num_partials > 1:
        if not a.is_contiguous() or a.shape[0] != num_partials or a.shape[-1] != 256:
            raise RuntimeError("row_seg: partials must be a contiguous [S, rows, 256] tensor")
        g.a, g.ld_a, g.partial_stride = ctypes.c_void_p(a.data_ptr()), 256, a.numel() // num_partials
        keep.append(a)
    else:
        if a.shape[-1] != 256:
            raise RuntimeError("row_seg: segments are 256 wide")
        t, g.a, g.ld_a = _rows2d(a, "a")
        g.partial_stride = 0
        keep.append(t)
    g.num_partials, g.a_scale, g.relu = num_partials, float(a_scale), int(relu)
    if bias0 is not None:
        g.bias0 = ctypes.c_void_p(bias0.data_ptr())
        keep.append(bias0)
    if residual is not None:
        t, g.residual, g.ld_res = _rows2d(residual, "residual")
        keep.append(t)
    if norm is not None:
        g.gamma, g.beta, g.eps = ctypes.c_void_p(norm.weight.data_ptr()), ctypes.c_void_p(norm.bias.data_ptr()), float(norm.eps)
    if post is not None:
        t, g.post, g.ld_post = _rows2d(post, "post")
        keep.append(t)
    if x_out is not None:
        t, g.x_out, g.ld_xout = _rows2d(x_out, "x_out")
        keep.append(t)
    if split_out is not None:
        width = 512 if split_lines else 768 + SPLIT_BIAS_PAD
        if split_out.dtype != torch.float16 or not split_out.is_contiguous() or split_out.shape[-1] != width:
            raise RuntimeError(f"row_seg: split_out must be a contiguous f16 [rows, {width}] tensor")
        g.split_out, g.split_scale = ctypes.c_void_p(split_out.data_ptr()), SPLIT_ACT_SCALE
        g.split_pad, g.split_layout = (0, 1) if split_lines else (SPLIT_BIAS_PAD, 0)
        keep.append(split_out)
    g._keep = keep
    return g


def row_gemm(segs, weight, bias, out, relu_from=None):
    d = _lib.RowGemm()
    N, K = weight.shape
    if K != 256 * len(segs) or not weight.is_contiguous() or not weight.is_cuda or weight.dtype != torch.float32:
        raise RuntimeError("row_gemm: weight must be a contiguous float32 CUDA [N, 256 * segments] tensor")
    for i, g in enumerate(segs):
        d.seg[i] = g
    d.num_seg, d.N = len(segs), N
    d.w = ctypes.c_void_p(weight.data_ptr())
    d.b = ctypes.c_void_p(bias.data_ptr()) if bias is not None else None
    t, d.out, d.ld_out = _rows2d(out, "out")
    if out.shape[-1] != N:
        raise RuntimeError("row_gemm: out must be [rows, N]")
    d.relu_from = N if relu_from is None else int(relu_from)
    d._keep = [segs, weight, bias, t]
    return d


def rowgemm_launch(descs, rows):
    arr = (_lib.RowGemm * len(descs))(*descs)
    rc = _lib.lib().rac_rowgemm_fwd(arr, len(descs), int(rows), _lib.stream_ptr())
    _lib.check(rc, "rac_rowgemm_fwd")


def pack_gemm_split_weight(weight):
    import math
    w = weight.detach().float().contiguous()
    N, K = w.shape
    amax = float(w.abs().max())
    if K % 32 != 0 or not w.is_cuda or not (amax > 0.0) or amax != amax or amax == float("inf"):
        return None, None
    s = 13 - math.frexp(amax)[1] + 1
    img = torch.empty(N, K // 32, 64, device=w.device, dtype=torch.float16)
    _lib.check(_lib.lib().rac_gemm_split_pack_fwd(_lib.ptr(w), _lib.ptr(img), N, K, float(2.0 ** s), _lib.stream_ptr()),
               "rac_gemm_split_pack_fwd")
    return img, 2.0 ** (-s) / SPLIT_ACT_SCALE


def value_proj_fused(maps, w_image, w_alpha, add=None, bias=None, q16=False):
    _lib.require_gpu(maps, w_image, what="value_proj_fused")
    F_, C, H, W = maps.shape
    if maps.dtype != torch.float32 or not maps.is_contiguous() or w_image.dtype != torch.float16 or tuple(w_image.shape) != (256, 8, 64):
        raise RuntimeError("value_proj_fused: maps must be contiguous float32 [F,256,H,W], w_image f16 [256,8,64]")
    if add is not None and (add.dtype != torch.float32 or not add.is_contiguous() or tuple(add.shape) != (H * W, 256)):
        raise RuntimeError("value_proj_fused: add must be a contiguous float32 [H*W, 256] tensor")
    if q16:
        out = torch.empty(F_, H * W, 4, 64, device=maps.device, dtype=torch.int16)
        scale = torch.empty(F_, H * W, 4, device=maps.device, dtype=torch.float32)
    else:
        out = torch.empty(F_, H * W, 256, device=maps.device, dtype=torch.float32)
    ev = _lib.timer.record("value_proj_fwd") if _lib.timer is not None else None
    if ev:
        ev[0].record()
    head = (_lib.ptr(maps), _lib.ptr(w_image), float(w_alpha), _lib.ptr(add) if add is not None else None,
            _lib.ptr(bias) if bias is not None else None)
    tail = (F_, C, H * W, 256, _lib.stream_ptr())
    if q16:
        rc, what = _lib.lib().rac_value_proj_q16_fwd(*head, _lib.ptr(out), _lib.ptr(scale), *tail), "rac_value_proj_q16_fwd"
    else:
        rc, what = _lib.lib().rac_value_proj_fwd(*head, _lib.ptr(out), *tail), "rac_value_proj_fwd"
    if ev:
        ev[1].record()
    _lib.check(rc, what)
    return (out, scale) if q16 else out


def generator_fused(x_image, w_image, bias, alpha, timer_name="mixing_generator_gemm", ld_out=None):
    _lib.require_gpu(x_image, w_image, what="generator_fused")
    M = x_image.shape[0]
    N, lines, _ = w_image.shape
    if x_image.dtype != torch.float16 or w_image.dtype != torch.float16 or x_image.numel() != M * lines * 64 or w_image.shape[2] != 64:
        raise RuntimeError("generator_fused: operand images do not match")
    ld_out = N if ld_out is None else int(ld_out)
    out = torch.empty(M, ld_out, device=x_image.device, dtype=torch.float32)
    ev = _lib.timer.record(timer_name) if _lib.timer is not None and timer_name else None
    if ev:
        ev[0].record()
    rc = _lib.lib().rac_generator_fwd(_lib.ptr(x_image), _lib.ptr(w_image), _lib.ptr(bias) if bias is not None else None, float(alpha),
                                      _lib.ptr(out), ld_out, M, N, lines * 32, _lib.stream_ptr())
    if ev:
        ev[1].record()
    _lib.check(rc, "rac_generator_fwd")
    return out


def outproj_fused(z_image, w_image, slices):
    _lib.require_gpu(z_image, w_image, what="outproj_fused")
    M, lines, _ = z_image.shape
    N = w_image.shape[0]
    if z_image.dtype != torch.float16 or w_image.dtype != torch.float16 or tuple(w_image.shape[1:]) != (lines, 64) \
            or z_image.shape[2] != 64 or lines % slices != 0:
        raise RuntimeError("outproj_fused: operand images do not match")
    out = torch.empty(slices, M, N, device=z_image.device, dtype=torch.float32)
    ev = _lib.timer.record("mixing_out_proj_gemm") if _lib.timer is not None else None
    if ev:
        ev[0].record()
    rc = _lib.lib().rac_outproj_fwd(_lib.ptr(z_image), _lib.ptr(w_image), _lib.ptr(out), M, N, lines * 32, slices, _lib.stream_ptr())
    if ev:
        ev[1].record()
    _lib.check(rc, "rac_outproj_fwd")
    return out


def decode_fused(cls_scores, bbox_preds, max_num, post_center_range, score_threshold=None, out=None):
    cls_scores, bbox_preds = cls_scores.contiguous(), bbox_preds.contiguous()
    _lib.require_gpu(cls_scores, bbox_preds, what="decode_fused")
    Q, C = cls_scores.shape
    if out is None:
        out = torch.empty(max_num, 11, device=cls_scores.device, dtype=torch.float32)
    rng = (ctypes.c_float * 6)(*[float(v) for v in post_center_range])
    rc = _lib.lib().rac_decode_fwd(_lib.ptr(cls_scores), _lib.ptr(bbox_preds), _lib.ptr(out), Q, C, int(max_num), rng,
                                   float(score_threshold or 0.0), int(bool(score_threshold)), _lib.stream_ptr())
    _lib.check(rc, "rac_decode_fwd")
    return out
```

### racformer_amd/transformer.py

```python
import math
import os

import numpy as np
import torch
import torch.nn as nn
import torch.nn.functional as F

from . import _lib
from .bbox_utils import decode_bbox, inverse_sigmoid, theta_d2xy_coods, xy2theta_d_coods
from .fused import (SPLIT_ACT_SCALE, SPLIT_BIAS_PAD, SPLIT_SLICE, ConvImage, act_image, add_ln, bev_sampling_fused, bev_sampling_multi_fused,
                    box_prep, conv_direct, quantize_values_i16, upsample2x_image,
                    generator_fused, gru_gate_fused, layer_boundary_fused, mixing_fused, mixing_sampled_fused, mixing_sampled_supported, outproj_fused,
                    pack_conv3x3_weight,
                    pack_gemm_split_weight,
                    pe_head, refine_fused, row_gemm,
                    row_seg, rowgemm_launch, sampling4d_fused, sasa_fused, split_weight_f16, upsample2x_fused, value_proj_fused)
from .msda import msda_forward
from .msmv import msmv_forward

try:
    from mmdet.models.utils.builder import TRANSFORMER as _TRANSFORMER
    _register = _TRANSFORMER.register_module()
except Exception:
    def _register(cls):
        return cls

_TWO_PI = 2 * math.pi

_ALTERNATE_PLANS = {}


def register_alternate_plan(name, fn):
    _ALTERNATE_PLANS[name] = fn


def alternate_plan(name):
    if name not in _ALTERNATE_PLANS:
        raise RuntimeError(f"execution plan '{name}' is a cross-check of the parity tests: import tests/plans.py to register it")
    return _ALTERNATE_PLANS[name]


class _AttnParams(nn.Module):

    def __init__(self, embed_dims):
        super().__init__()
        self.in_proj_weight = nn.Parameter(torch.empty(3 * embed_dims, embed_dims))
        self.in_proj_bias = nn.Parameter(torch.zeros(3 * embed_dims))
        self.out_proj = nn.Linear(embed_dims, embed_dims)
        nn.init.xavier_uniform_(self.in_proj_weight)


class _MHAHolder(nn.Module):

    def __init__(self, embed_dims):
        super().__init__()
        self.attn = _AttnParams(embed_dims)


class _FFN(nn.Module):

    def __init__(self, embed_dims, feedforward_channels):
        super().__init__()
        self.layers = nn.Sequential(
            nn.Sequential(nn.Linear(embed_dims, feedforward_channels), nn.ReLU(inplace=True), nn.Dropout(0.0)),
            nn.Linear(feedforward_channels, embed_dims), nn.Dropout(0.0))

    def forward(self, x):
        return x + self.layers(x)


class _LearnedPositionalEncoding(nn.Module):

    def __init__(self, num_feats, row_num_embed, col_num_embed):
        super().__init__()
        self.row_embed = nn.Embedding(row_num_embed, num_feats)
        self.col_embed = nn.Embedding(col_num_embed, num_feats)

    def grid(self, h, w):
        col = self.col_embed.weight[:w]
        row = self.row_embed.weight[:h]
        pos = torch.cat([col[None].expand(h, w, -1), row[:, None].expand(h, w, -1)], dim=-1)
        return pos.permute(2, 0, 1)


class ScaleAdaptiveSelfAttention(nn.Module):

    def __init__(self, embed_dims=256, num_heads=8, dropout=0.1, pc_range=[], init_cfg=None):
        super().__init__()
        self.pc_range = pc_range
        self.embed_dims = embed_dims
        self.num_heads = num_heads
        self.attention = _MHAHolder(embed_dims)
        self.gen_tau = nn.Linear(embed_dims, num_heads)
        self.fused = True

    @torch.no_grad()
    def init_weights(self):
        nn.init.zeros_(self.gen_tau.weight)
        nn.init.uniform_(self.gen_tau.bias, 0.0, 2.0)

    def wide_in_proj(self):
        p = self.attention.attn
        return (torch.cat([p.in_proj_weight, self.gen_tau.weight], dim=0),
                torch.cat([p.in_proj_bias, self.gen_tau.bias], dim=0))

    def forward(self, query_bbox, query_feat, pre_attn_mask=None, prepared_w=None):
        if self.fused and pre_attn_mask is None and self.embed_dims // self.num_heads == 32:
            p = self.attention.attn
            if prepared_w is None:
                prepared_w = self.wide_in_proj()
            lin = F.linear(query_feat, prepared_w[0], prepared_w[1])
            E = self.embed_dims
            o = sasa_fused(lin[..., :3 * E], lin[..., 3 * E:], query_bbox.contiguous(), self.num_heads, self.pc_range)
            return query_feat + p.out_proj(o)
        return self.forward_unfused(query_bbox, query_feat, pre_attn_mask)

    def forward_unfused(self, query_bbox, query_feat, pre_attn_mask=None):
        B, Q, E = query_feat.shape
        Hn, d = self.num_heads, E // self.num_heads
        centers = decode_bbox(theta_d2xy_coods(query_bbox), self.pc_range)[..., :2]
        dist = -torch.cdist(centers, centers, compute_mode="donot_use_mm_for_euclid_dist")
        tau = self.gen_tau(query_feat).permute(0, 2, 1)
        mask = dist[:, None] * tau[..., None]
        if pre_attn_mask is not None:
            mask[:, :, pre_attn_mask] = float("-inf")
        p = self.attention.attn
        qkv = F.linear(query_feat, p.in_proj_weight, p.in_proj_bias).view(B, Q, 3, Hn, d)
        q = qkv[:, :, 0].permute(0, 2, 1, 3) * math.sqrt(1.0 / d)
        k = qkv[:, :, 1].permute(0, 2, 1, 3)
        v = qkv[:, :, 2].permute(0, 2, 1, 3)
        attn = torch.softmax(mask + q @ k.transpose(-1, -2), dim=-1)
        o = (attn @ v).permute(0, 2, 1, 3).reshape(B, Q, E)
        return query_feat + p.out_proj(o)


def make_sample_points(query_bbox, offset, pc_range):
    d = decode_bbox(query_bbox, pc_range)
    xyz, wlh, ang = d[..., 0:3], d[..., 3:6], d[..., 6:7]
    delta = wlh[:, :, None, :] * offset[..., 0:3]
    c, s = torch.cos(ang)[..., None, :], torch.sin(ang)[..., None, :]
    rot = torch.cat([delta[..., 0:1] * c - delta[..., 1:2] * s,
                     delta[..., 0:1] * s + delta[..., 1:2] * c, delta[..., 2:3]], dim=-1)
    return xyz[:, :, None, :] + rot


COMPACT_BELOW_COVERAGE = 0.8


def compact_variant(coverage):
    return None if coverage is None else bool(coverage < COMPACT_BELOW_COVERAGE)


def rig_coverage(lidar2img, num_cams, image_hw, pc_range):
    l2i = np.asarray(lidar2img, dtype=np.float64).reshape(-1, 4, 4)[:num_cams]
    H, W = image_hw
    az = np.linspace(0.0, 2.0 * np.pi, 72, endpoint=False)
    rmax = 0.9 * min(abs(pc_range[0]), abs(pc_range[1]), pc_range[3], pc_range[4])
    pts = np.array([[r * np.cos(a), r * np.sin(a), z, 1.0] for a in az for r in (0.15 * rmax, 0.4 * rmax, 0.7 * rmax, rmax) for z in (0.0, 1.5)])
    cam = np.einsum("nij,pj->npi", l2i, pts)
    z = cam[..., 2]
    with np.errstate(divide="ignore", invalid="ignore"):
        u, v = cam[..., 0] / np.maximum(z, 1e-5) / W, cam[..., 1] / np.maximum(z, 1e-5) / H
    seen = (z > 1e-5) & (u > 0) & (u < 1) & (v > 0) & (v < 1)
    return float(seen.any(axis=0).mean())


def _warp_to_polar(points_xy, vel, time_diff, pc_range):
    shift = (vel[:, :, None, :] * time_diff[:, None, :, None])[:, :, :, None, None, :]
    xy = points_xy - shift
    x = (xy[..., 0:1] - pc_range[0]) / (pc_range[3] - pc_range[0])
    y = (xy[..., 1:2] - pc_range[1]) / (pc_range[4] - pc_range[1])
    pol = xy2theta_d_coods(torch.cat([x, y], dim=-1))
    return pol[..., 0:1], pol[..., 1:2]


class RaCFormerSampling(nn.Module):

    def __init__(self, embed_dims=256, num_frames=4, num_groups=4, num_points=8, num_levels=4,
                 depth_num=15, pc_range=[], init_cfg=None):
        super().__init__()
        self.num_frames, self.num_points, self.num_groups = num_frames, num_points, num_groups
        self.num_levels, self.pc_range, self.depth_num = num_levels, pc_range, depth_num
        self.ray_points_offset = nn.Linear(embed_dims, depth_num)
        self.sampling_offset = nn.Linear(embed_dims, depth_num * num_groups * num_points * 3)
        self.scale_weights = nn.Linear(embed_dims, num_groups * num_frames * depth_num * num_points * num_levels)
        self.capture_loc = None
        self.force_views = None
        self.force_views_cyclic = False
        self._force_i = 0
        self._last_forced = None

    def _next_forced(self):
        self._last_forced = None
        if not self.force_views:
            return None
        if self.force_views_cyclic:
            v = self.force_views[self._force_i % len(self.force_views)]
            self._force_i += 1
        else:
            v = self.force_views.pop(0)
        self._last_forced = v
        return v

    def init_weights(self):
        bias = self.sampling_offset.bias.data.view(self.depth_num * self.num_groups * self.num_points, 3)
        nn.init.zeros_(self.sampling_offset.weight)
        nn.init.uniform_(bias[:, 0:3], -0.5, 0.5)

    def forward(self, query_ray, query_feat, mlvl_feats, img_metas, d_region=0.1, linear_out=None, debug=False,
                box_table=None):
        image_h, image_w, _ = img_metas[0]["img_shape"][0]
        if linear_out is None:
            linear_out = (self.sampling_offset(query_feat), self.ray_points_offset(query_feat),
                          self.scale_weights(query_feat))
        off, ray, sc = linear_out
        res = sampling4d_fused(mlvl_feats, query_ray.contiguous(), off, ray, sc, img_metas[0]["time_diff"],
                               img_metas[0]["lidar2img"], self.num_frames, self.num_groups, self.num_points,
                               self.depth_num, self.pc_range, d_region, image_h, image_w,
                               debug=debug or self.capture_loc is not None, box_table=box_table, view_in=self._next_forced(),
                               compact=compact_variant(img_metas[0].get("_rac_coverage")))
        if self.capture_loc is not None:
            self.capture_loc.append(res[1])
            return res if debug else res[0]
        return res


    def forward_into_mixing(self, query_ray, mlvl_feats, img_metas, d_region, linear_out, box_table, params, out_points=128):
        image_h, image_w, _ = img_metas[0]["img_shape"][0]
        off, ray, sc = linear_out
        res = mixing_sampled_fused(mlvl_feats, query_ray.contiguous(), off, ray, sc, img_metas[0]["time_diff"], img_metas[0]["lidar2img"],
                                   self.num_frames, self.num_groups, self.num_points, self.depth_num, self.pc_range, d_region, image_h,
                                   image_w, params, out_points=out_points, debug=self.capture_loc is not None, box_table=box_table,
                                   view_in=self._next_forced())
        if self.capture_loc is not None:
            self.capture_loc.append(res[1])
            return res[0]
        return res


def sampling_4d(sample_points, mlvl_feats, scale_weights, lidar2img, image_h, image_w, aggregate=True,
                eps=1e-5, loc_tap=None, view_in=None):
    if not aggregate:
        raise NotImplementedError("sampling_4d(aggregate=False) is not on the inference path")
    B, Q, T, G, P, _ = sample_points.shape
    N = lidar2img.shape[1] // T
    m = lidar2img.view(B, T, N, 1, 1, 4, 4)
    p = sample_points.permute(0, 2, 1, 3, 4, 5).reshape(B, T, 1, Q, G * P, 3)
    x, y, z = p[..., 0], p[..., 1], p[..., 2]
    cx = m[..., 0, 0] * x + m[..., 0, 1] * y + m[..., 0, 2] * z + m[..., 0, 3]
    cy = m[..., 1, 0] * x + m[..., 1, 1] * y + m[..., 1, 2] * z + m[..., 1, 3]
    homo = m[..., 2, 0] * x + m[..., 2, 1] * y + m[..., 2, 2] * z + m[..., 2, 3]
    hz = torch.clamp(homo, min=eps)
    u = cx / hz / image_w
    v = cy / hz / image_h
    valid = (homo > eps) & (v > 0.0) & (v < 1.0) & (u > 0.0) & (u < 1.0)
    i_view = own_view = torch.argmax(valid.to(torch.uint8), dim=2, keepdim=True)
    if view_in is not None:
        i_view = view_in.long().view(B, T, G, Q, P).permute(0, 1, 3, 2, 4).reshape(B, T, 1, Q, G * P)
    u_sel = torch.gather(u, 2, i_view)[:, :, 0]
    v_sel = torch.gather(v, 2, i_view)[:, :, 0]
    loc = torch.stack([u_sel, v_sel, i_view[:, :, 0].to(u.dtype) / (N - 1)], dim=-1)
    loc = loc.view(B, T, Q, G, P, 3).permute(0, 1, 3, 2, 4, 5).reshape(B * T * G, Q, P, 3).contiguous()
    if loc_tap is not None:
        own = torch.stack([u_sel, v_sel, own_view[:, :, 0].to(u.dtype) / (N - 1)], dim=-1)
        loc_tap.append(own.view(B, T, Q, G, P, 3).permute(0, 1, 3, 2, 4, 5).reshape(B * T * G, Q, P, 3))
    L = scale_weights.shape[-1]
    w = scale_weights.reshape(B, Q, G, T, P, L).permute(0, 2, 3, 1, 4, 5).reshape(B * G * T, Q, P, L).contiguous()
    return msmv_forward(mlvl_feats, loc, w, out_layout=_lib.OUT_BQGTPC, num_frames=T, num_groups=G)


class ConvGRUCell(nn.Module):
    def __init__(self, input_channels, hidden_channels, kernel_size):
        super().__init__()
        self.hidden_channels = hidden_channels
        self.gates_conv = nn.Conv2d(input_channels + hidden_channels, 3 * hidden_channels,
                                    kernel_size=kernel_size, padding=kernel_size // 2)
        self.matching_layer = nn.Conv2d(hidden_channels, input_channels, 1)

    def gates(self, x, h_prev):
        return self.gates_conv(torch.cat([x, self.matching_layer(h_prev)], dim=1))

    def forward(self, x, h_prev):
        gates = self.gates(x, h_prev)
        z_gate, r_gate, cand = torch.split(gates, self.hidden_channels, dim=1)
        z, r = torch.sigmoid(z_gate), torch.sigmoid(r_gate)
        cand = torch.tanh(cand + r * h_prev)
        return (1 - z) * h_prev + z * cand


class ConvGRU(nn.Module):

    def __init__(self, input_channels, hidden_channels, kernel_size):
        super().__init__()
        self.convGRUCell = ConvGRUCell(input_channels, hidden_channels, kernel_size)
        self.hidden_channels = hidden_channels

    def forward(self, x):
        B, T, C, H, W = x.shape
        h = torch.zeros(B, self.hidden_channels, H, W, device=x.device, dtype=x.dtype)
        out = torch.zeros(B, T, self.hidden_channels, H, W, device=x.device, dtype=x.dtype)
        fused = x.is_cuda and x.dtype == torch.float32 and (self.hidden_channels * H * W) % 4 == 0
        for t in range(min(4, T)):
            if fused:
                h = gru_gate_fused(self.convGRUCell.gates(x[:, t], h), h, out[:, t])
            else:
                h = self.convGRUCell(x[:, t], h)
                out[:, t] = h
        return out


def convgru_fused_pack(gru, h, w):
    cell = gru.convGRUCell
    C = cell.hidden_channels
    dev = cell.gates_conv.weight.device
    wg = cell.gates_conv.weight.detach().double().cpu()
    bg = cell.gates_conv.bias.detach().double().cpu() if cell.gates_conv.bias is not None else wg.new_zeros(wg.shape[0])
    m = cell.matching_layer.weight.detach().double().cpu()[:, :, 0, 0]
    bm = cell.matching_layer.bias.detach().double().cpu() if cell.matching_layer.bias is not None else m.new_zeros(m.shape[0])
    if wg.shape[1] != 2 * C or m.shape != (C, C):
# ... 409 lines not shown
        assert G == self.n_groups and P == self.in_points and C == self.eff_in_dim
        params = self.parameter_generator(query)
        if out_proj_split is not None and self.fused_supported(x):
            out = mixing_fused(x.contiguous(), params, P, G, self.out_points)
            S_, N, k = out_proj_split.shape
            a3 = out.view(B * Q, S_, k).transpose(0, 1)
            proj = torch.bmm(a3, out_proj_split.transpose(1, 2)).sum(0) + self.out_proj.bias
            return query + proj.view(B, Q, N)
        params = params.reshape(B * Q, G, -1)
        M, S = params.split([self.m_parameters, self.s_parameters], 2)
        M = M.reshape(B * Q, G, self.eff_in_dim, self.eff_out_dim)
        S = S.reshape(B * Q, G, self.out_points, self.in_points)
        out = torch.matmul(x.reshape(B * Q, G, P, C), M)
        out = F.relu(F.layer_norm(out, [out.size(-2), out.size(-1)]))
        out = torch.matmul(S, out)
        out = F.relu(F.layer_norm(out, [out.size(-2), out.size(-1)]))
        if out_proj_split is None:
            return query + self.out_proj(out.reshape(B, Q, -1))
        S, N, k = out_proj_split.shape
        a3 = out.reshape(B * Q, S, k).transpose(0, 1)
        proj = torch.bmm(a3, out_proj_split.transpose(1, 2)).sum(0) + self.out_proj.bias
        return query + proj.view(B, Q, N)


class RaCFormerTransformerDecoderLayer(nn.Module):

    def __init__(self, embed_dims, num_frames=8, num_points=4, num_points_bev=4, num_levels=4, num_classes=10,
                 code_size=10, num_cls_fcs=2, num_reg_fcs=2, img_depth_num=3, bev_depth_num=5, num_ray=150,
                 pc_range=[], d_region_list=[0.15, 0.1, 0.1, 0.08, 0.08, 0.05], spatial_shapes=(128, 128),
                 init_cfg=None):
        super().__init__()
        self.embed_dims, self.num_classes, self.code_size, self.pc_range = embed_dims, num_classes, code_size, pc_range
        self.position_encoder = nn.Sequential(
            nn.Linear(3, embed_dims), nn.LayerNorm(embed_dims), nn.ReLU(inplace=True),
            nn.Linear(embed_dims, embed_dims), nn.LayerNorm(embed_dims), nn.ReLU(inplace=True))
        self.self_attn = ScaleAdaptiveSelfAttention(embed_dims, num_heads=8, dropout=0.1, pc_range=pc_range)
        self.sampling = RaCFormerSampling(embed_dims, num_frames=num_frames, num_groups=4, num_points=num_points,
                                          num_levels=num_levels, depth_num=img_depth_num, pc_range=pc_range)
        self.sampling_radar_bev = BEVSampling(embed_dims, num_frames=num_frames, num_heads=4,
                                              num_points=num_points_bev, num_levels=1, pc_range=pc_range,
                                              depth_num=bev_depth_num, spatial_shapes=spatial_shapes,
                                              temp_radar=True)
        self.sampling_lss_bev = BEVSampling(embed_dims, num_frames=num_frames, num_heads=4,
                                            num_points=num_points_bev, num_levels=1, pc_range=pc_range,
                                            depth_num=bev_depth_num, spatial_shapes=spatial_shapes)
        self.mixing = AdaptiveMixing(in_dim=embed_dims, in_points=num_points * num_frames * img_depth_num,
                                     n_groups=4, out_points=128)
        self.ffn = _FFN(embed_dims, 512)
        self.norm1 = nn.LayerNorm(embed_dims)
        self.norm2 = nn.LayerNorm(embed_dims)
        self.norm3 = nn.LayerNorm(embed_dims)
        self.fusion = nn.Linear(embed_dims * 3, embed_dims)
        self.norm_radar_bev = nn.LayerNorm(embed_dims)
        self.norm_lss_bev = nn.LayerNorm(embed_dims)
        self.norm_fusion = nn.LayerNorm(embed_dims)
        cls_branch = []
        for _ in range(num_cls_fcs):
            cls_branch += [nn.Linear(embed_dims, embed_dims), nn.LayerNorm(embed_dims), nn.ReLU(inplace=True)]
        cls_branch.append(nn.Linear(embed_dims, num_classes))
        self.cls_branch = nn.Sequential(*cls_branch)
        reg_branch = []
        for _ in range(num_reg_fcs):
            reg_branch += [nn.Linear(embed_dims, embed_dims), nn.ReLU(inplace=True)]
        reg_branch.append(nn.Linear(embed_dims, code_size))
        self.reg_branch = nn.Sequential(*reg_branch)
        self.d_region_list = d_region_list
        self.num_ray = num_ray
        self.fused = True
        self.split_gemm = True
        self.rowgemm = True
        self.own_generator = True
        self._carry = None
        self.compose_radar_value = True
        self.value_storage = "f32"
        self.fuse_sampling_mixing = os.environ.get("RAC_FUSE_SAMPLING_MIXING", "0") == "1"
        self.fused_q16_producers = True
        self._pack_cache = {}

    def _cached(self, key, params, fn):
        sig = tuple((p.data_ptr(), p._version, str(p.device)) for p in params)
        hit = self._pack_cache.get(key)
        if hit is None or hit[0] != sig:
            with torch.no_grad():
                hit = (sig, fn())
            self._pack_cache[key] = hit
        return hit[1]

    @torch.no_grad()
    def init_weights(self):
        self.self_attn.init_weights()
        self.sampling.init_weights()
        self.mixing.init_weights()
        self.sampling_radar_bev.init_weights()
        self.sampling_lss_bev.init_weights()
        nn.init.constant_(self.cls_branch[-1].bias, float(-math.log((1 - 0.01) / 0.01)))
        nn.init.xavier_uniform_(self.fusion.weight)
        nn.init.constant_(self.fusion.bias, 0.0)

    def mfma_report(self, cfg, split):
        Qn, E, G_, C_ = cfg.num_query, cfg.embed_dims, cfg.num_groups, cfg.channels
        Pin = cfg.num_points * cfg.num_frames * cfg.img_depth_num
        gen_cols = G_ * (C_ * C_ + 128 * Pin)
        bev_h, bev_w = cfg.bev_hw
        conv = 2.0 * cfg.num_frames * bev_h * bev_w * 256 * 320 * 9
        return [
            ("mixing_fwd", "mixing_c64_f16x3_kernel (hand-written; x@M: 6 bf16 products, S@Y: 3 f16 products)" if split
             else "mixing_c64_kernel (hand-written, v_mfma_f32_16x16x4_f32)",
             2.0 * Qn * G_ * (Pin * C_ * C_ + 128 * Pin * C_),
             2.0 * Qn * G_ * (6 * 96 * C_ * C_ + 3 * 128 * 96 * C_) if split else 2.0 * Qn * G_ * (96 * C_ * C_ + 128 * 96 * C_),
             16 if split else 32),
            ("mixing_sampled_fwd", "mixing_c64_f16x3_kernel<4> (the same two products; the workgroup gathers its own sampled features first: "
             "rac_mixing_sampled_fwd)", 2.0 * Qn * G_ * (Pin * C_ * C_ + 128 * Pin * C_),
             2.0 * Qn * G_ * (6 * 96 * C_ * C_ + 3 * 128 * 96 * C_), 16),
            ("mixing_generator_gemm", ("gemm_split_kernel (hand-written, 3 f16 products, loader waves + LDS-DMA ring)" if self.own_generator
                                       else "parameter_generator GEMM (hipBLASLt f16, K-concatenated hi/lo operands)") if split
             else "parameter_generator GEMM (rocBLAS fp32)",
             2.0 * Qn * E * gen_cols, 2.0 * Qn * gen_cols * ((3 * E + (0 if self.own_generator else 64)) if split else E),
             16 if split else 32),
            ("mixing_out_proj_gemm", "gemm_split_kernel (hand-written split-K GEMM, 3 f16 products, LDS-DMA staging)" if split
             else "out_proj split-K batched GEMM (rocBLAS fp32)",
             2.0 * Qn * (G_ * 128 * C_) * E, 2.0 * Qn * (G_ * 128 * C_) * E * (3 if split else 1), 16 if split else 32),
            ("temporal_fusion_conv", "conv3x3_f16x3_kernel (hand-written implicit GEMM, 3 f16 products; value_proj composed in)",
             conv, 3 * conv, 16)]

    def refine_bbox(self, bbox_proposal, bbox_delta):
        dz_new = torch.sigmoid(bbox_delta[..., 1:3] + inverse_sigmoid(bbox_proposal[..., 1:3]))
        theta = bbox_proposal[..., 0:1] + (torch.sigmoid(bbox_delta[..., 0:1]) * 2 - 1) / self.num_ray
        return torch.cat([theta, dz_new, bbox_delta[..., 3:]], dim=-1)

    def _sample(self, qb, x1, mlvl_feats, img_metas, d_region, linear_out, table):
        return self.sampling(qb, x1, mlvl_feats, img_metas, d_region=d_region, linear_out=linear_out, box_table=table)

    def _wide_linears(self):
        mods = [self.sampling.sampling_offset, self.sampling.ray_points_offset, self.sampling.scale_weights]
        for x in (self.sampling_radar_bev, self.sampling_lss_bev):
            mods += [x.sampling_offset, x.ray_points_offset, x.scale_weights, x.attention.bev_queue_weight]
        w = torch.cat([m.weight for m in mods], dim=0)
        b = torch.cat([m.bias for m in mods], dim=0)
        widths = [m.weight.shape[0] for m in mods]
        return w, b, widths

    def prepare(self, lss_bev_feats, radar_bev_feats):
        if self.value_storage not in ("f32", "i16"):
            raise RuntimeError(f"value_storage must be 'f32' or 'i16', got {self.value_storage!r}")
        rb_, lb_ = self.sampling_radar_bev, self.sampling_lss_bev
        i16 = (self.value_storage == "i16" and self.fused and self.rowgemm and radar_bev_feats.is_cuda and lss_bev_feats.is_cuda
               and radar_bev_feats.dtype == torch.float32 and lss_bev_feats.dtype == torch.float32
               and tuple(radar_bev_feats.shape) == tuple(lss_bev_feats.shape)
               and (rb_.num_frames, rb_.num_heads, rb_.num_points, rb_.depth_num) == (lb_.num_frames, lb_.num_heads, lb_.num_points, lb_.depth_num)
               and self.embed_dims == 64 * rb_.attention.num_heads == 64 * lb_.attention.num_heads)
        want_q16 = i16 and self.fused_q16_producers
        rbs = self.sampling_radar_bev
        te, up = rbs.temporal_encoder, rbs.temporal_encoder.upsample[1]
        conv_pack = None
        if radar_bev_feats.is_cuda and self.fused and te.fused_conv:
            Hr, Wr = radar_bev_feats.shape[-2:]
            cell = te.convGRU.convGRUCell
            conv_params = [te.temporal_fusion.weight, up.weight, te.downsample.weight, cell.gates_conv.weight,
                           cell.matching_layer.weight] + \
                [m.bias for m in (te.temporal_fusion, up, cell.gates_conv, cell.matching_layer, te.downsample) if m.bias is not None]
            if self.compose_radar_value:
                pe_, vp = rbs.positional_encoding, rbs.attention.value_proj
                conv_pack = self._cached(f"conv_value_pack_{Hr}x{Wr}", conv_params + [vp.weight, vp.bias, pe_.row_embed.weight,
                                                                                     pe_.col_embed.weight],
                                         lambda: rbs.composed_value_pack(Hr, Wr))
            if not conv_pack:
                def plain_pack():
                    ws, alpha = pack_conv3x3_weight(te.temporal_fusion.weight)
                    return dict(ws=ws, alpha=alpha, bound=te.hidden_bound(), **te.temporal_bias_maps(Hr, Wr), **te.downsample_pack(Hr, Wr))
                conv_pack = self._cached(f"conv_pack_{Hr}x{Wr}", conv_params, plain_pack)
        lbs = self.sampling_lss_bev
        if lss_bev_feats.is_cuda and self.fused:
            Hl, Wl = lss_bev_feats.shape[-2:]
            lvp, lpe = lbs.attention.value_proj, lbs.positional_encoding
            pos_term = self._cached(f"lss_pos_term_{Hl}x{Wl}", [lvp.weight, lvp.bias, lpe.row_embed.weight, lpe.col_embed.weight],
                                    lambda: lvp(lpe.grid(Hl, Wl).to(lvp.weight.dtype).reshape(-1, Hl * Wl).t()).contiguous())
            Bl, Tl, Cl = lss_bev_feats.shape[:3]
            vp_img = self._cached("lss_vp_img", [lvp.weight], lambda: pack_gemm_split_weight(lvp.weight)) \
                if Cl == 256 and lvp.weight.shape[0] == 256 and (Hl * Wl) % 32 == 0 and lss_bev_feats.dtype == torch.float32 \
                else (None, None)
            if vp_img[0] is not None:
                lss_value = value_proj_fused(lss_bev_feats.reshape(Bl * Tl, Cl, Hl, Wl).contiguous(), vp_img[0], vp_img[1] * SPLIT_ACT_SCALE,
                                             add=pos_term, q16=want_q16 and lbs.attention.num_heads == 4)
                if not isinstance(lss_value, tuple):
                    lss_value = lss_value.view(Bl * Tl, Hl * Wl, lbs.attention.num_heads, -1)
            else:
                lss_value = lbs.attention.project_value(lss_bev_feats, pos_term=pos_term)
            lss_hw = (Hl, Wl)
        else:
            lss_value, lss_hw = lbs.prepare_value(lss_bev_feats)
        radar_value, radar_hw = self.sampling_radar_bev.prepare_value(radar_bev_feats, conv_pack, q16=want_q16)
        rb, lb, mix = self.sampling_radar_bev, self.sampling_lss_bev, self.mixing
        wide_mods = [self.sampling.sampling_offset, self.sampling.ray_points_offset, self.sampling.scale_weights]
        for x in (rb, lb):
            wide_mods += [x.sampling_offset, x.ray_points_offset, x.scale_weights, x.attention.bev_queue_weight]
        w, b, widths = self._cached("wide", [p for m in wide_mods for p in (m.weight, m.bias)], self._wide_linears)
        ro, lo = rb.attention.output_proj, lb.attention.output_proj
        bev_owt, bev_ob = self._cached("bev_o", [ro.weight, lo.weight, ro.bias, lo.bias], lambda: (
            torch.stack([ro.weight.t(), lo.weight.t()]).contiguous(), torch.stack([ro.bias, lo.bias])[:, None, :].contiguous()))
        c0, r0 = self.cls_branch[0], self.reg_branch[0]
        c0r0_w, c0r0_b = self._cached("c0r0", [c0.weight, r0.weight, c0.bias, r0.bias], lambda: (
            torch.cat([c0.weight, r0.weight], dim=0), torch.cat([c0.bias, r0.bias], dim=0)))
        at = self.self_attn
        sasa_w = self._cached("sasa", [at.attention.attn.in_proj_weight, at.gen_tau.weight, at.attention.attn.in_proj_bias,
                                       at.gen_tau.bias], at.wide_in_proj)
        E_ = self.embed_dims
        w2_ = self.ffn.layers[1]
        kslices = self._cached("kslices", [self.fusion.weight, w2_.weight], lambda: (
            [self.fusion.weight[:, i * E_:(i + 1) * E_].contiguous() for i in range(self.fusion.weight.shape[1] // E_)],
            [w2_.weight[:, i * E_:(i + 1) * E_].contiguous() for i in range(w2_.weight.shape[1] // E_)]))
        packs = {}
        if self.split_gemm and radar_bev_feats.is_cuda and self.fused:
            packs = self._cached("split_packs", [mix.parameter_generator.weight, mix.parameter_generator.bias,
                                                 mix.out_proj.weight, self.norm1.weight, self.norm1.bias], lambda: mix.split_packs(
                float(self.norm1.weight.abs().max()) * math.sqrt(self.embed_dims) + float(self.norm1.bias.abs().max())))
        wide_img = self._cached("wide_img", [w], lambda: pack_gemm_split_weight(w)) if packs and self.own_generator else (None, None)
        out_proj_split = None if packs else self._cached("out_proj_split", [mix.out_proj.weight], mix.split_out_proj)
        value_scales = None
        if i16:
            (radar_value, rsc), (lss_value, lsc) = [v if isinstance(v, tuple) else quantize_values_i16(v.contiguous())
                                                    for v in (radar_value, lss_value)]
            value_scales = (rsc, lsc)
        return dict(radar_value=radar_value, radar_hw=radar_hw, lss_value=lss_value, lss_hw=lss_hw, value_scales=value_scales,
                    wide_w=w, wide_b=b, wide_widths=widths, wide_img=wide_img, out_proj_split=out_proj_split, split_packs=packs,
                    sasa_w=sasa_w, bev_owt=bev_owt, bev_ob=bev_ob, c0r0_w=c0r0_w, c0r0_b=c0r0_b,
                    fusion_k=kslices[0], ffn2_k=kslices[1])

    def forward_fused(self, query_bbox, query_feat, mlvl_feats, img_metas, layer, prepared, stages=None, out_slots=None):
        if not self.rowgemm:
            return alternate_plan("library_chain")(self, query_bbox, query_feat, mlvl_feats, img_metas, layer, prepared, stages)
        self.wrote_slots = False
        meta = img_metas[0]
        time_diff, d_region = meta["time_diff"], self.d_region_list[layer]
        qb = query_bbox.contiguous()
        B, Q, E = query_feat.shape
        n = B * Q
        dev = query_feat.device
        new = lambda *shape: torch.empty(*shape, device=dev, dtype=torch.float32)
        pe, p = self.position_encoder, self.self_attn.attention.attn
        packs = prepared.get("split_packs")
        carried = self._carry if self._carry is not None and self._carry[0] == (layer, qb.data_ptr(), tuple(qb.shape), qb._version) \
            else None
        self._carry = None
        h = carried[1] if carried is not None else pe_head(qb[..., :3], pe[0], pe[1])
        y2 = new(n, E)
        rowgemm_launch([row_gemm([row_seg(h)], pe[3].weight, pe[3].bias, y2)], n)
        x, lin = new(B, Q, E), new(B, Q, 3 * E + self.self_attn.num_heads)
        rowgemm_launch([row_gemm([row_seg(y2, norm=pe[4], relu=True, post=query_feat.contiguous(), x_out=x)],
                                 prepared["sasa_w"][0], prepared["sasa_w"][1], lin)], n)
        table = carried[2] if carried is not None else box_prep(qb, self.pc_range)
        o = sasa_fused(lin[..., :3 * E], lin[..., 3 * E:], qb, self.self_attn.num_heads, self.pc_range, box_table=table)
        attn = new(n, E)
        rowgemm_launch([row_gemm([row_seg(o)], p.out_proj.weight, p.out_proj.bias, attn)], n)
        x1 = new(B, Q, E)
        own_gen = bool(packs) and self.own_generator
        x1_split = torch.empty(n, 2 * E if own_gen else 3 * E + SPLIT_BIAS_PAD, device=dev, dtype=torch.float16) if packs else None
        wide_n = prepared["wide_w"].shape[0]
        wimg, walpha = prepared.get("wide_img", (None, None))
        if own_gen and wimg is not None:
            add_ln(attn.view(B, Q, E), self.norm1, residual=x, out=x1, split=True, split_lines=True, split_out=x1_split)
            wide = generator_fused(x1_split, wimg, prepared["wide_b"], walpha, timer_name=None, ld_out=(wide_n + 3) // 4 * 4)
            wide = wide.view(B, Q, -1)[..., :wide_n]
        else:
            wide = new(B, Q, wide_n)
            rowgemm_launch([row_gemm([row_seg(attn, residual=x, norm=self.norm1, x_out=x1, split_out=x1_split, split_lines=own_gen)],
                                     prepared["wide_w"], prepared["wide_b"], wide)], n)
        lin = wide.split(prepared["wide_widths"], dim=-1)
        rb, lb = self.sampling_radar_bev, self.sampling_lss_bev
        r_off, r_ray, r_sc, r_qu = lin[3:7]
        l_off, l_ray, l_sc, l_qu = lin[7:11]
        bev = new(2, B, Q, E)
        same = prepared["radar_hw"] == prepared["lss_hw"] and prepared["radar_value"].dtype == prepared["lss_value"].dtype and \
            (rb.num_frames, rb.num_heads, rb.num_points, rb.depth_num) == (lb.num_frames, lb.num_heads, lb.num_points, lb.depth_num)
        if same:
            bev_sampling_multi_fused([(prepared["radar_value"], r_off, r_ray, r_sc, r_qu), (prepared["lss_value"], l_off, l_ray, l_sc, l_qu)],
                                     prepared["radar_hw"], qb, time_diff, rb.num_frames, rb.num_heads, rb.num_points, rb.depth_num,
                                     rb.pc_range, d_region, table, bev, value_scales=prepared.get("value_scales"))
        elif prepared.get("value_scales") is not None:
            raise RuntimeError("value_storage='i16' is served by the two-stream launch only")
        else:
            bev_sampling_fused(prepared["radar_value"], prepared["radar_hw"], qb, r_off, r_ray, r_sc, r_qu, time_diff,
                               rb.num_frames, rb.num_heads, rb.num_points, rb.depth_num, rb.pc_range, d_region,
                               box_table=table, out=bev[0])
            bev_sampling_fused(prepared["lss_value"], prepared["lss_hw"], qb, l_off, l_ray, l_sc, l_qu, time_diff,
                               lb.num_frames, lb.num_heads, lb.num_points, lb.depth_num, lb.pc_range, d_region,
                               box_table=table, out=bev[1])
        smp, mix = self.sampling, self.mixing
        if (self.fuse_sampling_mixing and own_gen and mix.out_points == 128 and mix.eff_in_dim == 64 and mix.eff_out_dim == 64
                and mix.in_points == smp.num_frames * smp.num_points * smp.depth_num and smp.num_groups == mix.n_groups
                and mixing_sampled_supported(mlvl_feats, smp.num_frames, smp.num_points * smp.depth_num)):
            params = generator_fused(x1_split, packs["gen_img"], mix.parameter_generator.bias, packs["gen_img_alpha"]).view(B, Q, -1)
            img = smp.forward_into_mixing(qb, mlvl_feats, img_metas, d_region, lin[0:3], table, params, out_points=mix.out_points)
            partials = outproj_fused(img, packs["out_w"], packs["out_slices"])
            sampled_feat = None
            if stages is not None:
                image_h, image_w, _ = img_metas[0]["img_shape"][0]
                sampled_feat = sampling4d_fused(mlvl_feats, qb, *lin[0:3], img_metas[0]["time_diff"], img_metas[0]["lidar2img"], smp.num_frames,
                                                smp.num_groups, smp.num_points, smp.depth_num, smp.pc_range, d_region, image_h, image_w,
                                                box_table=table, view_in=smp._last_forced)
        else:
            sampled_feat = self._sample(qb, x1, mlvl_feats, img_metas, d_region, lin[0:3], table)
            partials = self.mixing.out_proj_partials(sampled_feat, x1, prepared["out_proj_split"], None, packs, x1_split)
        p_scale = packs["out_alpha"] if packs else 1.0
        proj = new(2, n, E)
        ro, lo = rb.attention.output_proj, lb.attention.output_proj
        rowgemm_launch([row_gemm([row_seg(bev[0])], ro.weight, ro.bias, proj[0]),
                        row_gemm([row_seg(bev[1])], lo.weight, lo.bias, proj[1])], n)
        x2 = add_ln(partials, self.norm2, residual=x1, bias=self.mixing.out_proj.bias, num_partials=partials.shape[0],
                    a_scale=p_scale)
        fk, f2k = prepared["fusion_k"], prepared["ffn2_k"]
        if len(fk) != 3 or len(f2k) != 2:
            raise RuntimeError("forward_fused: fusion must take 3 * embed_dims, feedforward_channels must be 2 * embed_dims")
        f_parts = new(3, n, E)
        rowgemm_launch([row_gemm([row_seg(x2)], fk[0], self.fusion.bias, f_parts[0]),
                        row_gemm([row_seg(proj[0], residual=x1, norm=self.norm_radar_bev)], fk[1], None, f_parts[1]),
                        row_gemm([row_seg(proj[1], residual=x1, norm=self.norm_lss_bev)], fk[2], None, f_parts[2])], n)
        f, h1, ffn_parts = new(n, E), new(n, 2 * E), new(2, n, E)
        w1, w2 = self.ffn.layers[0][0], self.ffn.layers[1]
        rowgemm_launch([row_gemm([row_seg(f_parts, num_partials=3, norm=self.norm_fusion, x_out=f)], w1.weight, w1.bias, h1, relu_from=0)], n)
        rowgemm_launch([row_gemm([row_seg(h1[:, :E])], f2k[0], w2.bias, ffn_parts[0]),
                        row_gemm([row_seg(h1[:, E:])], f2k[1], None, ffn_parts[1])], n)
        x3, c0r0 = new(B, Q, E), new(n, 2 * E)
        rowgemm_launch([row_gemm([row_seg(ffn_parts, num_partials=2, residual=f, norm=self.norm3, x_out=x3)], prepared["c0r0_w"],
                                 prepared["c0r0_b"], c0r0, relu_from=E)], n)
        cb, rg = self.cls_branch, self.reg_branch
        c3, r2 = new(n, E), new(n, E)
        rowgemm_launch([row_gemm([row_seg(c0r0[:, :E], norm=cb[1], relu=True)], cb[3].weight, cb[3].bias, c3),
                        row_gemm([row_seg(c0r0[:, E:])], rg[2].weight, rg[2].bias, r2, relu_from=0)], n)
        cls_score = out_slots[0] if out_slots is not None else new(B, Q, self.num_classes)
        delta = new(B, Q, self.code_size)
        rowgemm_launch([row_gemm([row_seg(c3, norm=cb[4], relu=True)], cb[6].weight, cb[6].bias, cls_score),
                        row_gemm([row_seg(r2)], rg[4].weight, rg[4].bias, delta)], n)
        bbox_pred, bbox_xy, next_table, next_h = layer_boundary_fused(qb, delta, meta["time_diff_safe"], self.num_ray,
                                                                      self.pc_range, pe[0], pe[1],
                                                                      xy_out=out_slots[1] if out_slots is not None else None)
        self.wrote_slots = out_slots is not None
        self._carry = ((layer + 1, bbox_pred.data_ptr(), tuple(bbox_pred.shape), bbox_pred._version), next_h, next_table, bbox_pred)
        if stages is not None:
            mixed = x1 + p_scale * partials.sum(0).view_as(x1) + self.mixing.out_proj.bias
            stages.update(position_encoder=x - query_feat, self_attn=x + attn.view_as(x),
                          sampling_radar_bev=proj[0].view_as(x1) + x1, sampling_lss_bev=proj[1].view_as(x1) + x1,
                          sampling=sampled_feat, mixing=mixed, ffn=(f + ffn_parts.sum(0)).view_as(x1))
        self.last_bbox_xy = bbox_xy
        return x3, cls_score, bbox_pred

    def forward(self, query_bbox, query_feat, mlvl_feats, lss_bev_feats, radar_bev_feats, attn_mask, img_metas,
                layer=0, prepared=None, stages=None, out_slots=None):
        if prepared is None:
            prepared = self.prepare(lss_bev_feats, radar_bev_feats)
        if not self.fused:
            return alternate_plan("reference_ops")(self, query_bbox, query_feat, mlvl_feats, attn_mask, img_metas, layer, prepared, stages)
        if attn_mask is None and query_feat.is_cuda and self.embed_dims == 256 and self.mixing.in_points <= 96:
            return self.forward_fused(query_bbox, query_feat, mlvl_feats, img_metas, layer, prepared, stages, out_slots)
        meta = img_metas[0]
        time_diff, d_region = meta["time_diff"], self.d_region_list[layer]
        query_pos = self.position_encoder(query_bbox[..., :3])
        query_feat = query_feat + query_pos
        sa = self.self_attn(query_bbox, query_feat, attn_mask, prepared.get("sasa_w"))
        query_feat = self.norm1(sa)
        lin = F.linear(query_feat, prepared["wide_w"], prepared["wide_b"]).split(prepared["wide_widths"], dim=-1)
        qb = query_bbox.contiguous()
        table = box_prep(qb, self.pc_range)
        radar_raw = self.sampling_radar_bev.attend_prepared(qb, query_feat, prepared["radar_value"],
                                                            prepared["radar_hw"], time_diff, d_region, lin[3:7], table)
        lss_raw = self.sampling_lss_bev.attend_prepared(qb, query_feat, prepared["lss_value"],
                                                        prepared["lss_hw"], time_diff, d_region, lin[7:11], table)
        sampled_feat = self._sample(qb, query_feat, mlvl_feats, img_metas, d_region, lin[0:3], table)
        query_radar_feat = self.norm_radar_bev(radar_raw)
        query_lss_feat = self.norm_lss_bev(lss_raw)
        mixed = self.mixing(sampled_feat, query_feat, prepared.get("out_proj_split"))
        query_feat = self.norm2(mixed)
        query_feat = self.norm_fusion(self.fusion(torch.cat((query_feat, query_radar_feat, query_lss_feat), dim=-1)))
        ffn_out = self.ffn(query_feat)
        query_feat = self.norm3(ffn_out)
        cls_score = self.cls_branch(query_feat)
        bbox_pred, bbox_xy = refine_fused(query_bbox, self.reg_branch(query_feat), meta["time_diff_safe"], self.num_ray)
        if stages is not None:
            stages.update(position_encoder=query_pos, self_attn=sa, sampling_radar_bev=radar_raw,
                          sampling_lss_bev=lss_raw, sampling=sampled_feat, mixing=mixed, ffn=ffn_out)
        self.last_bbox_xy = bbox_xy
        return query_feat, cls_score, bbox_pred


def regroup_pyramid(mlvl_feats, num_cams, groups=4, out_dtype=torch.float32):
    import ctypes
    feats, outs, dims = [], [], None
    for feat in mlvl_feats:
        B, TN, GC, H, W = feat.shape
        if TN % num_cams != 0 or GC % groups != 0:
            raise RuntimeError("regroup_pyramid: expected [B, T*N, G*C, H, W]")
        N, T, C = num_cams, TN // num_cams, GC // groups
        if dims is None:
            dims = (B, T, N, C)
        elif dims != (B, T, N, C):
            raise RuntimeError("regroup_pyramid: levels must share B, T*N and G*C")
        feat = feat.float().contiguous()
        _lib.require_gpu(feat, what="regroup_pyramid")
        feats.append(feat)
        outs.append(torch.empty(B * T * groups, N, H, W, C, device=feat.device, dtype=out_dtype))
    if not feats:
        return []
    B, T, N, C = dims
    code = _lib.RAC_F32 if out_dtype == torch.float32 else _lib.RAC_BF16
    if C % 4 == 0 and all((f.shape[3] * f.shape[4]) % 4 == 0 for f in feats) and len(feats) <= 8:
        L = len(feats)
        ins = (ctypes.c_void_p * L)(*[f.data_ptr() for f in feats])
        dst = (ctypes.c_void_p * L)(*[o.data_ptr() for o in outs])
        hw = (ctypes.c_int32 * (2 * L))(*[int(x) for f in feats for x in f.shape[3:5]])
        _lib.check(_lib.lib().rac_regroup_multi_fwd(L, ins, dst, hw, B, T, N, groups, C, code, _lib.stream_ptr()), "rac_regroup_multi_fwd")
        return outs
    for feat, dst in zip(feats, outs):
        H, W = feat.shape[3:5]
        _lib.check(_lib.lib().rac_regroup_fwd(_lib.ptr(feat), _lib.ptr(dst), B, T, N, groups, C, H, W, code, _lib.stream_ptr()),
                   "rac_regroup_fwd")
    return outs


class RaCFormerTransformerDecoder(nn.Module):

    def __init__(self, embed_dims, num_frames=8, num_points=4, num_points_bev=4, num_layers=6, num_levels=4,
                 num_classes=10, code_size=10, img_depth_num=3, bev_depth_num=5, pc_range=[], num_ray=150,
                 d_region_list=[0.15, 0.1, 0.1, 0.08, 0.08, 0.05], spatial_shapes=(128, 128), init_cfg=None,
                 num_cams=6):
        super().__init__()
        self.num_layers, self.pc_range, self.num_cams = num_layers, pc_range, num_cams
        self.decoder_layer = RaCFormerTransformerDecoderLayer(
            embed_dims, num_frames, num_points, num_points_bev, num_levels, num_classes, code_size,
            img_depth_num=img_depth_num, bev_depth_num=bev_depth_num, num_ray=num_ray, pc_range=pc_range,
            d_region_list=d_region_list, spatial_shapes=spatial_shapes)
        self.feature_dtype = torch.float32
        self.pregrouped = False

    @torch.no_grad()
    def init_weights(self):
        self.decoder_layer.init_weights()

    def stage_metas(self, img_metas, B, device):
        m0 = img_metas[0]
        ts = np.array([m["img_timestamp"] for m in img_metas], dtype=np.float64)
        l2i_staged = isinstance(m0.get("lidar2img"), torch.Tensor) and m0["lidar2img"].device == device \
            and m0["lidar2img"].dim() == 4 and m0["lidar2img"].shape[0] == B
        if l2i_staged and "time_diff_safe" in m0 and np.array_equal(m0.get("_rac_staged_ts"), ts):
            return
        m0["_rac_staged_ts"] = ts.copy()
        ts = np.reshape(ts, [B, -1, self.num_cams])
        td = np.mean(ts[:, :1, :] - ts, axis=-1).astype(np.float32)
        td_safe = td.copy()
        td_safe[td_safe < 1e-5] = 1.0
        parts = [td.ravel(), td_safe.ravel()]
        l2i = None
        if not l2i_staged:
            l2i = np.asarray([m["lidar2img"].cpu().numpy() if isinstance(m["lidar2img"], torch.Tensor) else m["lidar2img"]
                              for m in img_metas]).astype(np.float32)
            parts.append(l2i.ravel())
        flat = torch.from_numpy(np.concatenate(parts))
        if device.type == "cuda":
            dev = flat.pin_memory().to(device, non_blocking=True)
        else:
            dev = flat.to(device)
        n0, n1 = td.size, td.size + td_safe.size
        if l2i is not None and "img_shape" in m0:
            h_img, w_img = m0["img_shape"][0][:2]
            m0["_rac_coverage"] = rig_coverage(l2i[0], self.num_cams, (h_img, w_img), self.pc_range)
        m0["_rac_meta_block"] = dev if l2i is not None else None
        m0["time_diff"] = dev[:n0].view(td.shape)
        m0["time_diff_safe"] = dev[n0:n1].view(td_safe.shape)
        if l2i is not None:
            m0["lidar2img"] = dev[n1:].view(l2i.shape)

    def forward(self, query_bbox, query_feat, mlvl_feats, lss_bev_feats, radar_bev_feats, attn_mask, img_metas,
                stages_per_layer=None):
        self.stage_metas(img_metas, query_bbox.shape[0], query_bbox.device)
        if self.pregrouped:
            for f in mlvl_feats:
                if f.dim() != 5 or f.shape[1] != self.num_cams or not f.is_contiguous():
                    raise RuntimeError("pregrouped pyramid levels must be contiguous [B*T*G, N, H, W, C]")
        else:
            grouped = regroup_pyramid(mlvl_feats, self.num_cams, 4, self.feature_dtype)
            for lvl, g in enumerate(grouped):
                mlvl_feats[lvl] = g
        prepared = self.decoder_layer.prepare(lss_bev_feats, radar_bev_feats)
        self.decoder_layer._carry = None
        cls_scores, bbox_preds = [], []
        stacked = None
        if query_feat.is_cuda and not torch.is_grad_enabled():
            B, Q = query_bbox.shape[:2]
            dl = self.decoder_layer
            stacked = (torch.empty(self.num_layers, B, Q, dl.num_classes, device=query_feat.device, dtype=torch.float32),
                       torch.empty(self.num_layers, B, Q, dl.code_size, device=query_feat.device, dtype=torch.float32))
        for i in range(self.num_layers):
            st = {} if stages_per_layer is not None else None
            self.decoder_layer.wrote_slots = False
            query_feat, cls_score, bbox_pred = self.decoder_layer(
                query_bbox, query_feat, mlvl_feats, lss_bev_feats, radar_bev_feats, attn_mask, img_metas,
                layer=i, prepared=prepared, stages=st, out_slots=(stacked[0][i], stacked[1][i]) if stacked is not None else None)
            if stacked is not None and not self.decoder_layer.wrote_slots:
                stacked = None
            if stages_per_layer is not None:
                stages_per_layer.append(st)
            query_bbox = bbox_pred.detach()
            cls_scores.append(cls_score)
            bbox_preds.append(self.decoder_layer.last_bbox_xy)
        if stacked is not None:
            return stacked
        return torch.stack(cls_scores), torch.stack(bbox_preds)


@_register
class RaCFormerTransformer(nn.Module):

    def __init__(self, embed_dims, num_frames=8, num_points=4, num_points_bev=4, num_layers=6, num_levels=4,
                 num_classes=10, code_size=10, img_depth_num=3, bev_depth_num=5, pc_range=[], num_ray=150,
                 d_region_list=[0.15, 0.1, 0.1, 0.08, 0.08, 0.05], spatial_shapes=(128, 128), init_cfg=None,
                 num_cams=6):
        assert init_cfg is None, "To prevent abnormal initialization behavior, init_cfg is not allowed to be set"
        super().__init__()
        self.embed_dims, self.pc_range, self.num_cams = embed_dims, pc_range, num_cams
        self.decoder = RaCFormerTransformerDecoder(
            embed_dims, num_frames, num_points, num_points_bev, num_layers, num_levels, num_classes, code_size,
            img_depth_num=img_depth_num, bev_depth_num=bev_depth_num, pc_range=pc_range, num_ray=num_ray,
            d_region_list=d_region_list, spatial_shapes=spatial_shapes, num_cams=num_cams)

    @torch.no_grad()
    def init_weights(self):
        self.decoder.init_weights()

    def forward(self, query_bbox, query_feat, mlvl_feats, lss_bev_feats, radar_bev_feats, attn_mask, img_metas,
                stages_per_layer=None, raw=False):
        cls_scores, bbox_preds = self.decoder(query_bbox, query_feat, mlvl_feats, lss_bev_feats,
                                              radar_bev_feats, attn_mask, img_metas, stages_per_layer)
        if raw:
            return cls_scores, bbox_preds
        return torch.nan_to_num(cls_scores), torch.nan_to_num(bbox_preds)
```

Before: 272.9.

## Fuse add-LN into output-proj rowgemm and heads into layer-boundary kernel

Adds a rowgemm variant that also computes the norm2 add+LayerNorm over the mixing partials in the same launch as the BEV output projections. It also adds a fused kernel that runs the final cls/reg head GEMMs and then the layer-boundary box refinement with the PE linear+LN in one launch. Wave reductions switch from shfl_xor to permlane-swap/DPP builtins. The goal is to cut kernel launches and intermediate round trips per decoder layer, at the cost of more complex kernels and possible occupancy or register pressure changes.

```diff
diff --git a/include/racformer_hip.h b/include/racformer_hip.h
--- a/include/racformer_hip.h
+++ b/include/racformer_hip.h
@@ -7,7 +7,7 @@
 extern "C" {
 #endif
 
-#define RAC_ABI_VERSION 8
+#define RAC_ABI_VERSION 9
 #define RAC_MAX_LEVELS 8
 #define RAC_MAX_POINTS 128
 
@@ -165,6 +165,21 @@
     int num_seg, N, ld_out, relu_from;
 } rac_rowgemm;
 int rac_rowgemm_fwd(const rac_rowgemm *descs, int num, int rows, void *stream);
+
+typedef struct {
+    const float *a;
+    int64_t partial_stride;
+    const float *bias, *residual, *gamma, *beta;
+    float *out;
+    int ld_a, num_partials, ld_res, ld_out;
+    float a_scale, eps;
+} rac_rowln;
+int rac_rowgemm_ln_fwd(const rac_rowgemm *descs, int num, const rac_rowln *ln, int rows, void *stream);
+
+int rac_head_boundary_fwd(const rac_rowgemm *heads, const float *proposal, const float *time_diff_safe, float *bbox_pred,
+                          float *bbox_xy, float *box_table, const float *pc_range, const float *pe_weight, const float *pe_bias,
+                          const float *pe_gamma, const float *pe_beta, float *pe_out, int B, int Q, int T, int dim,
+                          float num_ray, float eps, void *stream);
 
 int rac_conv3x3s2_fwd(const void *xs, const void *ws, const float *bias, const float *amax, float w_alpha, float *out,
                       int out_channels_total, int N, int H, int W, int Cin, int Cin_image, int Cout, void *stream);
diff --git a/racformer_amd/_lib.py b/racformer_amd/_lib.py
--- a/racformer_amd/_lib.py
+++ b/racformer_amd/_lib.py
@@ -35,6 +35,8 @@
     "rac_sasa_fwd": (_i, [_vp] * 5 + [_i] * 6 + [_vp, _vp]),
     "rac_decode_fwd": (_i, [_vp, _vp, _vp, _i, _i, _i, _vp, _f, _i, _vp]),
     "rac_rowgemm_fwd": (_i, [_vp, _i, _i, _vp]),
+    "rac_rowgemm_ln_fwd": (_i, [_vp, _i, _vp, _i, _vp]),
+    "rac_head_boundary_fwd": (_i, [_vp] * 12 + [_i] * 4 + [_f, _f, _vp]),
     "rac_gemm_split_pack_fwd": (_i, [_vp, _vp, _i, _i, _f, _vp]),
     "rac_value_proj_fwd": (_i, [_vp, _vp, _f, _vp, _vp, _vp, _i, _i, _i, _i, _vp]),
     "rac_value_proj_q16_fwd": (_i, [_vp, _vp, _f, _vp, _vp, _vp, _vp, _i, _i, _i, _i, _vp]),
@@ -69,6 +71,11 @@
 class RowGemm(ctypes.Structure):
     _fields_ = [("seg", RowSeg * 3), ("w", _vp), ("b", _vp), ("out", _vp), ("num_seg", _i), ("N", _i), ("ld_out", _i),
                 ("relu_from", _i)]
+
+
+class RowLn(ctypes.Structure):
+    _fields_ = [("a", _vp), ("partial_stride", ctypes.c_int64), ("bias", _vp), ("residual", _vp), ("gamma", _vp), ("beta", _vp),
+                ("out", _vp), ("ld_a", _i), ("num_partials", _i), ("ld_res", _i), ("ld_out", _i), ("a_scale", _f), ("eps", _f)]
 
 
 class CdScale(ctypes.Structure):
diff --git a/racformer_amd/csrc/add_ln.hip b/racformer_amd/csrc/add_ln.hip
--- a/racformer_amd/csrc/add_ln.hip
+++ b/racformer_amd/csrc/add_ln.hip
@@ -2,13 +2,7 @@
 
 #define ALN_MAX_V 4
 
-__device__ __forceinline__ float aln_wave_sum(float v)
-{
-#pragma unroll
-    for (int off = 32; off >= 1; off >>= 1)
-        v += __shfl_xor(v, off, 64);
-    return v;
-}
+__device__ __forceinline__ float aln_wave_sum(float v) { return rac_wave_sum(v); }
 
 __global__ __launch_bounds__(256) void add_ln_kernel(const float *__restrict__ a, int S, long pstride, int ld_a, float a_scale,
                                                      const float *__restrict__ residual, const float *__restrict__ bias,
diff --git a/racformer_amd/csrc/boundary_device.h b/racformer_amd/csrc/boundary_device.h
--- /dev/null
+++ b/racformer_amd/csrc/boundary_device.h
@@ -0,0 +1,89 @@
+#pragma once
+#include "rac_common.h"
+
+#define REF_TWO_PI 6.283185307179586f
+
+__device__ __forceinline__ float ref_sigmoid(float x) { return 1.f / (1.f + expf(-x)); }
+
+__device__ __forceinline__ float ref_inverse_sigmoid(float x)
+{
+    x = fminf(fmaxf(x, 0.f), 1.f);
+    const float x1 = fmaxf(x, 1e-5f), x2 = fmaxf(1.f - x, 1e-5f);
+    return logf(x1 / x2);
+}
+
+__device__ __forceinline__ float lb_wave_sum(float v) { return rac_wave_sum(v); }
+
+struct rac_boundary_args {
+    const float *prop, *td_safe, *W, *bias, *gamma, *beta;
+    float *pred, *xy, *table, *h_out;
+    int Q, T;
+    float num_ray, eps, p0, p1, p2, sx, sy, sz;
+};
+
+__device__ __forceinline__ void rac_boundary_row(const rac_boundary_args &a, int i, const float *d, int lane)
+{
+    const float *p = a.prop + (size_t)i * 10;
+    float o[10];
+    o[0] = p[0] + (ref_sigmoid(d[0]) * 2.f - 1.f) / a.num_ray;
+    o[1] = ref_sigmoid(d[1] + ref_inverse_sigmoid(p[1]));
+    o[2] = ref_sigmoid(d[2] + ref_inverse_sigmoid(p[2]));
+#pragma unroll
+    for (int k = 3; k < 10; ++k)
+        o[k] = d[k];
+    if (a.T > 1) {
+        const float td = a.td_safe[(i / a.Q) * a.T + 1];
+        o[8] = o[8] / td;
+        o[9] = o[9] / td;
+    }
+    const float ang = o[0] * REF_TWO_PI, rad = o[1] * 65.0f;
+    const float xn = fminf(fmaxf((51.2f + rad * cosf(ang)) / 102.4f, 0.f), 1.f);
+    const float yn = fminf(fmaxf((51.2f + rad * sinf(ang)) / 102.4f, 0.f), 1.f);
+    if (lane == 0) {
+        float *pp = a.pred + (size_t)i * 10, *px = a.xy + (size_t)i * 10, *t = a.table + (size_t)i * 8;
+#pragma unroll
+        for (int k = 0; k < 10; ++k)
+            pp[k] = o[k];
+        px[0] = xn;
+        px[1] = yn;
+#pragma unroll
+        for (int k = 2; k < 10; ++k)
+            px[k] = o[k];
+        const float yaw = atan2f(o[6], o[7]);
+        t[0] = xn * a.sx + a.p0;
+        t[1] = yn * a.sy + a.p1;
+        t[2] = o[2] * a.sz + a.p2;
+        t[3] = expf(o[3]);
+        t[4] = expf(o[4]);
+        t[5] = expf(o[5]);
+        t[6] = cosf(yaw);
+        t[7] = sinf(yaw);
+    }
+    float v[4];
+#pragma unroll
+    for (int j = 0; j < 4; ++j) {
+        const int c = lane * 4 + j;
+        v[j] = a.W[c * 3] * o[0] + a.W[c * 3 + 1] * o[1] + a.W[c * 3 + 2] * o[2] + a.bias[c];
+    }
+    const float mean = lb_wave_sum((v[0] + v[1]) + (v[2] + v[3])) / 256.f;
+    const float d0 = v[0] - mean, d1 = v[1] - mean, d2 = v[2] - mean, d3 = v[3] - mean;
+    const float rstd = 1.f / sqrtf(lb_wave_sum((d0 * d0 + d1 * d1) + (d2 * d2 + d3 * d3)) / 256.f + a.eps);
+    const rac_f4 g = rac_ld4(a.gamma + lane * 4), b = rac_ld4(a.beta + lane * 4);
+    rac_f4 y = {fmaxf(d0 * rstd * g.x + b.x, 0.f), fmaxf(d1 * rstd * g.y + b.y, 0.f), fmaxf(d2 * rstd * g.z + b.z, 0.f),
+                fmaxf(d3 * rstd * g.w + b.w, 0.f)};
+    *reinterpret_cast<rac_f4 *>(a.h_out + (size_t)i * 256 + lane * 4) = y;
+}
+
+inline rac_boundary_args rac_make_boundary_args(const float *proposal, const float *time_diff_safe, float *bbox_pred, float *bbox_xy,
+                                                float *box_table, const float *pc_range, const float *pe_weight, const float *pe_bias,
+                                                const float *pe_gamma, const float *pe_beta, float *pe_out, int Q, int T, float num_ray,
+                                                float eps)
+{
+    rac_boundary_args a;
+    a.prop = proposal; a.td_safe = time_diff_safe; a.W = pe_weight; a.bias = pe_bias; a.gamma = pe_gamma; a.beta = pe_beta;
+    a.pred = bbox_pred; a.xy = bbox_xy; a.table = box_table; a.h_out = pe_out;
+    a.Q = Q; a.T = T; a.num_ray = num_ray; a.eps = eps;
+    a.p0 = pc_range[0]; a.p1 = pc_range[1]; a.p2 = pc_range[2];
+    a.sx = pc_range[3] - pc_range[0]; a.sy = pc_range[4] - pc_range[1]; a.sz = pc_range[5] - pc_range[2];
+    return a;
+}
diff --git a/racformer_amd/csrc/rac_common.h b/racformer_amd/csrc/rac_common.h
--- a/racformer_amd/csrc/rac_common.h
+++ b/racformer_amd/csrc/rac_common.h
@@ -48,6 +48,19 @@
 __device__ __forceinline__ float rac_bf16_to_f32(unsigned short v)
 {
     return __uint_as_float(((unsigned)v) << 16);
+}
+
+__device__ __forceinline__ float rac_wave_sum(float v)
+{
+    const auto h32 = __builtin_amdgcn_permlane32_swap(__float_as_uint(v), __float_as_uint(v), false, false);
+    v = __uint_as_float(h32[0]) + __uint_as_float(h32[1]);
+    const auto h16 = __builtin_amdgcn_permlane16_swap(__float_as_uint(v), __float_as_uint(v), false, false);
+    v = __uint_as_float(h16[0]) + __uint_as_float(h16[1]);
+    v += __int_as_float(__builtin_amdgcn_update_dpp(0, __float_as_int(v), 0x128, 0xf, 0xf, false));
+    v += __int_as_float(__builtin_amdgcn_update_dpp(0, __float_as_int(v), 0x124, 0xf, 0xf, false));
+    v += __int_as_float(__builtin_amdgcn_update_dpp(0, __float_as_int(v), 0x4E, 0xf, 0xf, false));
+    v += __int_as_float(__builtin_amdgcn_update_dpp(0, __float_as_int(v), 0xB1, 0xf, 0xf, false));
+    return v;
 }
 
 struct alignas(16) rac_f4 {
diff --git a/racformer_amd/csrc/refine.hip b/racformer_amd/csrc/refine.hip
--- a/racformer_amd/csrc/refine.hip
+++ b/racformer_amd/csrc/refine.hip
@@ -1,15 +1,4 @@
-#include "rac_common.h"
-
-#define REF_TWO_PI 6.283185307179586f
-
-__device__ __forceinline__ float ref_sigmoid(float x) { return 1.f / (1.f + expf(-x)); }
-
-__device__ __forceinline__ float ref_inverse_sigmoid(float x)
-{
-    x = fminf(fmaxf(x, 0.f), 1.f);
-    const float x1 = fmaxf(x, 1e-5f), x2 = fmaxf(1.f - x, 1e-5f);
-    return logf(x1 / x2);
-}
+#include "boundary_device.h"
 
 __global__ __launch_bounds__(256) void refine_kernel(const float *__restrict__ prop, const float *__restrict__ delta,
                                                      const float *__restrict__ td_safe, float *__restrict__ pred,
@@ -98,75 +87,12 @@
     return rac_launch_status("rac_head_finish_fwd");
 }
 
-__device__ __forceinline__ float lb_wave_sum(float v)
-{
-#pragma unroll
-    for (int off = 32; off >= 1; off >>= 1)
-        v += __shfl_xor(v, off, 64);
-    return v;
-}
-
-__global__ __launch_bounds__(256) void layer_boundary_kernel(const float *__restrict__ prop, const float *__restrict__ delta,
-                                                             const float *__restrict__ td_safe, float *__restrict__ pred,
-                                                             float *__restrict__ xy, float *__restrict__ table,
-                                                             const float *__restrict__ W, const float *__restrict__ bias,
-                                                             const float *__restrict__ gamma, const float *__restrict__ beta,
-                                                             float *__restrict__ h_out, int n, int Q, int T, float num_ray,
-                                                             float eps, float p0, float p1, float p2, float sx, float sy, float sz)
+__global__ __launch_bounds__(256) void layer_boundary_kernel(const rac_boundary_args a, const float *__restrict__ delta, int n)
 {
     const int i = blockIdx.x * 4 + (threadIdx.x >> 6);
-    const int lane = threadIdx.x & 63;
     if (i >= n)
         return;
-    const float *p = prop + (size_t)i * 10, *d = delta + (size_t)i * 10;
-    float o[10];
-    o[0] = p[0] + (ref_sigmoid(d[0]) * 2.f - 1.f) / num_ray;
-    o[1] = ref_sigmoid(d[1] + ref_inverse_sigmoid(p[1]));
-    o[2] = ref_sigmoid(d[2] + ref_inverse_sigmoid(p[2]));
-#pragma unroll
-    for (int k = 3; k < 10; ++k)
-        o[k] = d[k];
-    if (T > 1) {
-        const float td = td_safe[(i / Q) * T + 1];
-        o[8] = o[8] / td;
-        o[9] = o[9] / td;
-    }
-    const float ang = o[0] * REF_TWO_PI, rad = o[1] * 65.0f;
-    const float xn = fminf(fmaxf((51.2f + rad * cosf(ang)) / 102.4f, 0.f), 1.f);
-    const float yn = fminf(fmaxf((51.2f + rad * sinf(ang)) / 102.4f, 0.f), 1.f);
-    if (lane == 0) {
-        float *pp = pred + (size_t)i * 10, *px = xy + (size_t)i * 10, *t = table + (size_t)i * 8;
-#pragma unroll
-        for (int k = 0; k < 10; ++k)
-            pp[k] = o[k];
-        px[0] = xn;
-        px[1] = yn;
-#pragma unroll
-        for (int k = 2; k < 10; ++k)
-            px[k] = o[k];
-        const float yaw = atan2f(o[6], o[7]);
-        t[0] = xn * sx + p0;
-        t[1] = yn * sy + p1;
-        t[2] = o[2] * sz + p2;
-        t[3] = expf(o[3]);
-        t[4] = expf(o[4]);
-        t[5] = expf(o[5]);
-        t[6] = cosf(yaw);
-        t[7] = sinf(yaw);
-    }
-    float v[4];
-#pragma unroll
-    for (int j = 0; j < 4; ++j) {
-        const int c = lane * 4 + j;
-        v[j] = W[c * 3] * o[0] + W[c * 3 + 1] * o[1] + W[c * 3 + 2] * o[2] + bias[c];
-    }
-    const float mean = lb_wave_sum((v[0] + v[1]) + (v[2] + v[3])) / 256.f;
-    const float d0 = v[0] - mean, d1 = v[1] - mean, d2 = v[2] - mean, d3 = v[3] - mean;
-    const float rstd = 1.f / sqrtf(lb_wave_sum((d0 * d0 + d1 * d1) + (d2 * d2 + d3 * d3)) / 256.f + eps);
-    const rac_f4 g = rac_ld4(gamma + lane * 4), b = rac_ld4(beta + lane * 4);
-    rac_f4 y = {fmaxf(d0 * rstd * g.x + b.x, 0.f), fmaxf(d1 * rstd * g.y + b.y, 0.f), fmaxf(d2 * rstd * g.z + b.z, 0.f),
-                fmaxf(d3 * rstd * g.w + b.w, 0.f)};
-    *reinterpret_cast<rac_f4 *>(h_out + (size_t)i * 256 + lane * 4) = y;
+    rac_boundary_row(a, i, delta + (size_t)i * 10, threadIdx.x & 63);
 }
 
 extern "C" int rac_layer_boundary_fwd(const float *proposal, const float *delta, const float *time_diff_safe, float *bbox_pred,
@@ -181,9 +107,8 @@
                       pe_gamma && pe_beta && pe_out,
                   "rac_layer_boundary_fwd: null pointer");
     const int n = B * Q;
-    hipLaunchKernelGGL(layer_boundary_kernel, dim3((n + 3) / 4), dim3(256), 0, (hipStream_t)stream, proposal, delta,
-                       time_diff_safe, bbox_pred, bbox_xy, box_table, pe_weight, pe_bias, pe_gamma, pe_beta, pe_out, n, Q, T,
-                       num_ray, eps, pc_range[0], pc_range[1], pc_range[2], pc_range[3] - pc_range[0], pc_range[4] - pc_range[1],
-                       pc_range[5] - pc_range[2]);
+    const rac_boundary_args a = rac_make_boundary_args(proposal, time_diff_safe, bbox_pred, bbox_xy, box_table, pc_range, pe_weight,
+                                                       pe_bias, pe_gamma, pe_beta, pe_out, Q, T, num_ray, eps);
+    hipLaunchKernelGGL(layer_boundary_kernel, dim3((n + 3) / 4), dim3(256), 0, (hipStream_t)stream, a, delta, n);
     return rac_launch_status("rac_layer_boundary_fwd");
 }
diff --git a/racformer_amd/csrc/rowgemm.hip b/racformer_amd/csrc/rowgemm.hip
--- a/racformer_amd/csrc/rowgemm.hip
+++ b/racformer_amd/csrc/rowgemm.hip
@@ -1,39 +1,43 @@
 #include "rac_common.h"
+#include "boundary_device.h"
 
 typedef float rg_f4 __attribute__((ext_vector_type(4)));
 
 struct RowGemmArgs {
     rac_rowgemm d[RAC_ROWGEMM_MAX_BATCH];
-    int rows;
+    rac_rowln ln;
+    int rows, num;
 };
 
-__device__ __forceinline__ float rg_wave_sum(float v)
-{
-#pragma unroll
-    for (int off = 32; off >= 1; off >>= 1)
-        v += __shfl_xor(v, off, 64);
-    return v;
-}
-
-template <int NSEG, int MT, bool EARLY>
-__device__ __forceinline__ void rowgemm_body(const rac_rowgemm &d, int rows, float *sX)
-{
-    constexpr int K = 256 * NSEG, LD = K + 4, R = 16 * MT;
-    const int tid = threadIdx.x, wave = tid >> 6, lane = tid & 63;
-    const int row0 = blockIdx.x * R, n0 = blockIdx.y * 64;
-    const bool first_slice = blockIdx.y == 0;
-    const int li = lane & 15, lk = lane >> 4;
-    const int col = n0 + 16 * wave + li;
-    const int wrow = col < d.N ? col : d.N - 1;
-    const float *bp = d.w + (size_t)wrow * K + 4 * lk;
-    const int rot = (blockIdx.x * 5) & 15;
-    rac_f4 bcur[16], bnxt[16];
-    if (EARLY) {
-#pragma unroll
-        for (int u = 0; u < 16; ++u)
-            bcur[u] = rac_ld4(bp + 16 * ((u + rot) & 15));
-    }
-
+__device__ __forceinline__ float rg_wave_sum(float v) { return rac_wave_sum(v); }
+
+#if defined(RAC_DIAGNOSTIC_BUILD) && defined(RG_STAMPS)
+#define RG_STAMP_WGS 512
+__device__ unsigned long long rg_stamp_buf[RG_STAMP_WGS * 2 * 9];
+__device__ __forceinline__ void rg_stamp(int i, bool wait)
+{
+    if (wait)
+        asm volatile("s_waitcnt vmcnt(0)" ::: "memory");
+    const int wave = threadIdx.x >> 6, wg = blockIdx.x * gridDim.y + blockIdx.y;
+    if ((threadIdx.x & 63) == 0 && (wave == 0 || wave == 3) && wg < RG_STAMP_WGS && blockIdx.z == 0)
+        rg_stamp_buf[(wg * 2 + (wave != 0)) * 9 + i] = i == 8 ? __builtin_amdgcn_s_memrealtime() : __builtin_amdgcn_s_memtime();
+}
+#define RG_STAMP(i) rg_stamp(i, false)
+#define RG_STAMP_LANDED(i) rg_stamp(i, true)
+extern "C" int rac_dbg_rg_stamps(unsigned long long *host_out)
+{
+    hipDeviceSynchronize();
+    return (int)hipMemcpyFromSymbol(host_out, HIP_SYMBOL(rg_stamp_buf), sizeof(rg_stamp_buf), 0, hipMemcpyDeviceToHost);
+}
+#else
+#define RG_STAMP(i)
+#define RG_STAMP_LANDED(i)
+#endif
+
+template <int NSEG, int MT>
+__device__ __forceinline__ void rg_prologue(const rac_rowgemm &d, int rows, float *sX, int row0, int wave, int lane, bool first_slice)
+{
+    constexpr int K = 256 * NSEG, LD = K + 4;
 #pragma unroll
     for (int s = 0; s < NSEG; ++s) {
         const rac_rowseg &g = d.seg[s];
@@ -76,6 +80,8 @@
                     vv[rr].z += w[0][rr].z + w[1][rr].z; vv[rr].w += w[0][rr].w + w[1][rr].w;
                 }
             }
+            if (s == 0 && rb == 0)
+                RG_STAMP_LANDED(2);
 #pragma unroll
             for (int rr = 0; rr < 4; ++rr) {
                 const int r = rbase + rr, row = row0 + r;
@@ -125,15 +131,14 @@
             }
         }
     }
-    __syncthreads();
-
+}
+
+template <int NSEG, int MT>
+__device__ __forceinline__ void rg_mfma(const float *sX, const float *bp, int rot, int li, int lk, rac_f4 (&bcur)[16], rg_f4 (&acc)[MT][2])
+{
+    constexpr int LD = 256 * NSEG + 4;
     const float *ap = sX + li * LD + 4 * lk;
-    if (!EARLY) {
-#pragma unroll
-        for (int u = 0; u < 16; ++u)
-            bcur[u] = rac_ld4(bp + 16 * ((u + rot) & 15));
-    }
-    rg_f4 acc[MT][2];
+    rac_f4 bnxt[16];
 #pragma unroll
     for (int m = 0; m < MT; ++m)
         acc[m][0] = acc[m][1] = (rg_f4){0.f, 0.f, 0.f, 0.f};
@@ -162,6 +167,39 @@
                 bcur[u] = bnxt[u];
         }
     }
+}
+
+template <int NSEG, int MT, bool EARLY>
+__device__ __forceinline__ void rowgemm_body(const rac_rowgemm &d, int rows, float *sX)
+{
+    constexpr int K = 256 * NSEG, R = 16 * MT;
+    const int tid = threadIdx.x, wave = tid >> 6, lane = tid & 63;
+    const int row0 = blockIdx.x * R, n0 = blockIdx.y * 64;
+    const int li = lane & 15, lk = lane >> 4;
+    const int col = n0 + 16 * wave + li;
+    const int wrow = col < d.N ? col : d.N - 1;
+    const float *bp = d.w + (size_t)wrow * K + 4 * lk;
+    const int rot = (blockIdx.x * 5) & 15;
+    rac_f4 bcur[16];
+    if (EARLY) {
+#pragma unroll
+        for (int u = 0; u < 16; ++u)
+            bcur[u] = rac_ld4(bp + 16 * ((u + rot) & 15));
+    }
+    RG_STAMP(1);
+    rg_prologue<NSEG, MT>(d, rows, sX, row0, wave, lane, blockIdx.y == 0);
+    RG_STAMP(3);
+    __syncthreads();
+    RG_STAMP(4);
+    if (!EARLY) {
+#pragma unroll
+        for (int u = 0; u < 16; ++u)
+            bcur[u] = rac_ld4(bp + 16 * ((u + rot) & 15));
+    }
+    RG_STAMP_LANDED(5);
+    rg_f4 acc[MT][2];
+    rg_mfma<NSEG, MT>(sX, bp, rot, li, lk, bcur, acc);
+    RG_STAMP(6);
     const float bv = d.b ? d.b[wrow] : 0.f;
     const bool relu = col >= d.relu_from;
 #pragma unroll
@@ -175,56 +213,233 @@
             if (row < rows && col < d.N)
                 d.out[(size_t)row * d.ld_out + col] = v;
         }
-}
-
-template <int NSEG, int MT, bool EARLY>
+    RG_STAMP(7);
+    RG_STAMP(8);
+}
+
+__device__ __forceinline__ void rg_rowln(const rac_rowln &ln, int rows)
+{
+    const int wave = threadIdx.x >> 6, lane = threadIdx.x & 63;
+    const int S = ln.num_partials, per = (S + 3) / 4;
+    for (int r = blockIdx.y * 4 + wave; r < 16; r += 4 * gridDim.y) {
+        const int row = blockIdx.x * 16 + r;
+        if (row >= rows)
+            return;
+        rac_f4 q[4];
+#pragma unroll
+        for (int k = 0; k < 4; ++k)
+            q[k] = (rac_f4){0.f, 0.f, 0.f, 0.f};
+        for (int c0 = 0; c0 < per; c0 += 8) {
+            rac_f4 w[4][8];
+#pragma unroll
+            for (int k = 0; k < 4; ++k)
+#pragma unroll
+                for (int j = 0; j < 8; ++j) {
+                    const int s_lo = k * per, s_hi = min(S, s_lo + per);
+                    w[k][j] = (rac_f4){0.f, 0.f, 0.f, 0.f};
+                    if (s_lo + c0 + j < s_hi)
+                        w[k][j] = rac_ld4(ln.a + (size_t)(s_lo + c0 + j) * ln.partial_stride + (size_t)row * ln.ld_a + lane * 4);
+                }
+#pragma unroll
+            for (int k = 0; k < 4; ++k)
+                if (k * per + c0 < min(S, k * per + per)) {
+#pragma unroll
+                    for (int j = 0; j < 8; ++j) {
+                        q[k].x += w[k][j].x; q[k].y += w[k][j].y; q[k].z += w[k][j].z; q[k].w += w[k][j].w;
+                    }
+                }
+        }
+        rac_f4 v = q[0];
+#pragma unroll
+        for (int k = 1; k < 4; ++k) {
+            v.x += q[k].x; v.y += q[k].y; v.z += q[k].z; v.w += q[k].w;
+        }
+        v.x *= ln.a_scale; v.y *= ln.a_scale; v.z *= ln.a_scale; v.w *= ln.a_scale;
+        if (ln.bias) {
+            const rac_f4 w = rac_ld4(ln.bias + lane * 4);
+            v.x += w.x; v.y += w.y; v.z += w.z; v.w += w.w;
+        }
+        if (ln.residual) {
+            const rac_f4 w = rac_ld4(ln.residual + (size_t)row * ln.ld_res + lane * 4);
+            v.x += w.x; v.y += w.y; v.z += w.z; v.w += w.w;
+        }
+        const float mean = rg_wave_sum((v.x + v.y) + (v.z + v.w)) / 256.f;
+        const float d0 = v.x - mean, d1 = v.y - mean, d2 = v.z - mean, d3 = v.w - mean;
+        const float rstd = 1.f / sqrtf(rg_wave_sum((d0 * d0 + d1 * d1) + (d2 * d2 + d3 * d3)) / 256.f + ln.eps);
+        const rac_f4 g = rac_ld4(ln.gamma + lane * 4), b = rac_ld4(ln.beta + lane * 4);
+        const rac_f4 y = {d0 * rstd * g.x + b.x, d1 * rstd * g.y + b.y, d2 * rstd * g.z + b.z, d3 * rstd * g.w + b.w};
+        *reinterpret_cast<rac_f4 *>(ln.out + (size_t)row * ln.ld_out + lane * 4) = y;
+    }
+}
+
+template <int NSEG, int MT, bool EARLY, bool LNJOB>
 __global__ __launch_bounds__(256, EARLY ? 2 : 4) void rowgemm_kernel(const RowGemmArgs a)
 {
     extern __shared__ float smem[];
+    RG_STAMP(0);
+    if (LNJOB && (int)blockIdx.z == a.num) {
+        rg_rowln(a.ln, a.rows);
+        return;
+    }
     const rac_rowgemm &d = a.d[blockIdx.z];
     if ((int)blockIdx.y * 64 >= d.N)
         return;
     rowgemm_body<NSEG, MT, EARLY>(d, a.rows, smem);
 }
 
-extern "C" int rac_rowgemm_fwd(const rac_rowgemm *descs, int num, int rows, void *stream)
-{
-    RAC_CHECK_ARG(descs && num >= 1 && num <= RAC_ROWGEMM_MAX_BATCH && rows >= 0, "rac_rowgemm_fwd: num=%d rows=%d", num, rows);
-    if (rows == 0)
-        return 0;
+struct HeadBoundaryArgs {
+    rac_rowgemm d[2];
+    rac_boundary_args b;
+    int rows;
+};
+
+__global__ __launch_bounds__(256) void head_boundary_kernel(const HeadBoundaryArgs a)
+{
+    __shared__ float sX[2][16 * 260];
+    __shared__ float sD[16][16];
+    const int tid = threadIdx.x, wave = tid >> 6, lane = tid & 63;
+    const int li = lane & 15, lk = lane >> 4;
+    const int row0 = blockIdx.x * 16, rot = (blockIdx.x * 5) & 15;
+    const int h = wave & 1;
+    const rac_rowgemm &d = a.d[h];
+    const int wrow = li < d.N ? li : d.N - 1;
+    const float *bp = d.w + (size_t)wrow * 256 + 4 * lk;
+    rac_f4 bcur[16];
+    if (wave < 2) {
+#pragma unroll
+        for (int u = 0; u < 16; ++u)
+            bcur[u] = rac_ld4(bp + 16 * ((u + rot) & 15));
+    }
+    rg_prologue<1, 1>(a.d[0], a.rows, sX[0], row0, wave, lane, true);
+    rg_prologue<1, 1>(a.d[1], a.rows, sX[1], row0, wave, lane, true);
+    __syncthreads();
+    if (wave < 2) {
+        rg_f4 acc[1][2];
+        rg_mfma<1, 1>(sX[h], bp, rot, li, lk, bcur, acc);
+        const float bv = d.b ? d.b[wrow] : 0.f;
+        const bool relu = li >= d.relu_from;
+#pragma unroll
+        for (int r = 0; r < 4; ++r) {
+            const int row = row0 + 4 * lk + r;
+            float v = (acc[0][0][r] + acc[0][1][r]) + bv;
+            if (relu)
+                v = fmaxf(v, 0.f);
+            if (row < a.rows && li < d.N)
+                d.out[(size_t)row * d.ld_out + li] = v;
+            if (h == 1)
+                sD[4 * lk + r][li] = v;
+        }
+    }
+    __syncthreads();
+#pragma unroll
+    for (int k = 0; k < 4; ++k) {
+        const int r = wave * 4 + k;
+        if (row0 + r < a.rows)
+            rac_boundary_row(a.b, row0 + r, sD[r], lane);
+    }
+}
+
+static int rg_check_desc(const rac_rowgemm &d, int i, const char *who)
+{
+    RAC_CHECK_ARG(d.num_seg >= 1 && d.num_seg <= 3 && d.N >= 1 && d.w && d.out && d.ld_out >= d.N,
+                  "%s: GEMM %d: num_seg=%d N=%d ld_out=%d", who, i, d.num_seg, d.N, d.ld_out);
+    for (int s = 0; s < d.num_seg; ++s) {
+        const rac_rowseg &g = d.seg[s];
+        RAC_CHECK_ARG(g.a && g.ld_a >= 256 && g.ld_a % 4 == 0 && g.num_partials >= 1 && g.partial_stride % 4 == 0,
+                      "%s: GEMM %d segment %d: source rows (ld_a=%d, partials=%d)", who, i, s, g.ld_a, g.num_partials);
+        RAC_CHECK_ARG((!g.gamma) == (!g.beta), "%s: GEMM %d segment %d: gamma / beta must come together", who, i, s);
+        RAC_CHECK_ARG((!g.residual || g.ld_res % 4 == 0) && (!g.post || g.ld_post % 4 == 0) && (!g.x_out || g.ld_xout % 4 == 0),
+                      "%s: GEMM %d segment %d: row strides must be multiples of 4", who, i, s);
+        RAC_CHECK_ARG(!g.split_out || (g.split_pad >= 0 && g.split_pad <= 64 && g.split_pad % 4 == 0),
+                      "%s: GEMM %d segment %d: split_pad=%d", who, i, s, g.split_pad);
+    }
+    return 0;
+}
+
+static int rg_launch(const rac_rowgemm *descs, int num, const rac_rowln *ln, int rows, void *stream, const char *who)
+{
     RowGemmArgs a;
     int max_n = 0, max_seg = 0;
     for (int i = 0; i < num; ++i) {
         const rac_rowgemm &d = descs[i];
-        RAC_CHECK_ARG(d.num_seg >= 1 && d.num_seg <= 3 && d.N >= 1 && d.w && d.out && d.ld_out >= d.N,
-                      "rac_rowgemm_fwd: GEMM %d: num_seg=%d N=%d ld_out=%d", i, d.num_seg, d.N, d.ld_out);
-        for (int s = 0; s < d.num_seg; ++s) {
-            const rac_rowseg &g = d.seg[s];
-            RAC_CHECK_ARG(g.a && g.ld_a >= 256 && g.ld_a % 4 == 0 && g.num_partials >= 1 && g.partial_stride % 4 == 0,
-                          "rac_rowgemm_fwd: GEMM %d segment %d: source rows (ld_a=%d, partials=%d)", i, s, g.ld_a, g.num_partials);
-            RAC_CHECK_ARG((!g.gamma) == (!g.beta), "rac_rowgemm_fwd: GEMM %d segment %d: gamma / beta must come together", i, s);
-            RAC_CHECK_ARG((!g.residual || g.ld_res % 4 == 0) && (!g.post || g.ld_post % 4 == 0) && (!g.x_out || g.ld_xout % 4 == 0),
-                          "rac_rowgemm_fwd: GEMM %d segment %d: row strides must be multiples of 4", i, s);
-            RAC_CHECK_ARG(!g.split_out || (g.split_pad >= 0 && g.split_pad <= 64 && g.split_pad % 4 == 0),
-                          "rac_rowgemm_fwd: GEMM %d segment %d: split_pad=%d", i, s, g.split_pad);
-        }
-        RAC_CHECK_ARG(d.num_seg == descs[0].num_seg, "rac_rowgemm_fwd: batched GEMMs must have the same number of segments");
+        const int rc = rg_check_desc(d, i, who);
+        if (rc)
+            return rc;
+        RAC_CHECK_ARG(d.num_seg == descs[0].num_seg, "%s: batched GEMMs must have the same number of segments", who);
         a.d[i] = d;
         max_n = d.N > max_n ? d.N : max_n;
         max_seg = d.num_seg > max_seg ? d.num_seg : max_seg;
     }
     a.rows = rows;
+    a.num = num;
+    if (ln)
+        a.ln = *ln;
     hipStream_t st = (hipStream_t)stream;
     const int R = 16;
     const size_t lds = (size_t)R * (256 * max_seg + 4) * sizeof(float);
-    const dim3 grid((rows + R - 1) / R, (max_n + 63) / 64, num);
-    if (max_seg == 1 && (long)grid.x * grid.y * grid.z > 512)
-        hipLaunchKernelGGL((rowgemm_kernel<1, 1, false>), grid, dim3(256), lds, st, a);
+    const dim3 grid((rows + R - 1) / R, (max_n + 63) / 64, num + (ln ? 1 : 0));
+    if (ln)
+        hipLaunchKernelGGL((rowgemm_kernel<1, 1, true, true>), grid, dim3(256), lds, st, a);
+    else if (max_seg == 1 && (long)grid.x * grid.y * grid.z > 512)
+        hipLaunchKernelGGL((rowgemm_kernel<1, 1, false, false>), grid, dim3(256), lds, st, a);
     else if (max_seg == 1)
-        hipLaunchKernelGGL((rowgemm_kernel<1, 1, true>), grid, dim3(256), lds, st, a);
+        hipLaunchKernelGGL((rowgemm_kernel<1, 1, true, false>), grid, dim3(256), lds, st, a);
     else if (max_seg == 2)
-        hipLaunchKernelGGL((rowgemm_kernel<2, 1, true>), grid, dim3(256), lds, st, a);
+        hipLaunchKernelGGL((rowgemm_kernel<2, 1, true, false>), grid, dim3(256), lds, st, a);
     else
-        hipLaunchKernelGGL((rowgemm_kernel<3, 1, true>), grid, dim3(256), lds, st, a);
-    return rac_launch_status("rac_rowgemm_fwd");
-}
+        hipLaunchKernelGGL((rowgemm_kernel<3, 1, true, false>), grid, dim3(256), lds, st, a);
+    return rac_launch_status(who);
+}
+
+extern "C" int rac_rowgemm_fwd(const rac_rowgemm *descs, int num, int rows, void *stream)
+{
+    RAC_CHECK_ARG(descs && num >= 1 && num <= RAC_ROWGEMM_MAX_BATCH && rows >= 0, "rac_rowgemm_fwd: num=%d rows=%d", num, rows);
+    if (rows == 0)
+        return 0;
+    return rg_launch(descs, num, nullptr, rows, stream, "rac_rowgemm_fwd");
+}
+
+extern "C" int rac_rowgemm_ln_fwd(const rac_rowgemm *descs, int num, const rac_rowln *ln, int rows, void *stream)
+{
+    RAC_CHECK_ARG(descs && ln && num >= 1 && num <= RAC_ROWGEMM_MAX_BATCH && rows >= 0, "rac_rowgemm_ln_fwd: num=%d rows=%d", num, rows);
+    if (rows == 0)
+        return 0;
+    for (int i = 0; i < num; ++i)
+        RAC_CHECK_ARG(descs[i].num_seg == 1, "rac_rowgemm_ln_fwd: GEMM %d: num_seg=%d (the batch beside a row job is single-segment)", i,
+                      descs[i].num_seg);
+    RAC_CHECK_ARG(ln->a && ln->gamma && ln->beta && ln->out && ln->num_partials >= 1 && ln->ld_a >= 256 && ln->ld_a % 4 == 0 &&
+                      ln->partial_stride % 4 == 0 && ln->ld_out >= 256 && ln->ld_out % 4 == 0 && (!ln->residual || ln->ld_res % 4 == 0),
+                  "rac_rowgemm_ln_fwd: row job (partials=%d ld_a=%d ld_out=%d)", ln->num_partials, ln->ld_a, ln->ld_out);
+    return rg_launch(descs, num, ln, rows, stream, "rac_rowgemm_ln_fwd");
+}
+
+extern "C" int rac_head_boundary_fwd(const rac_rowgemm *heads, const float *proposal, const float *time_diff_safe, float *bbox_pred,
+                                     float *bbox_xy, float *box_table, const float *pc_range, const float *pe_weight, const float *pe_bias,
+                                     const float *pe_gamma, const float *pe_beta, float *pe_out, int B, int Q, int T, int dim,
+                                     float num_ray, float eps, void *stream)
+{
+    RAC_CHECK_ARG(heads && B >= 0 && Q >= 0 && T >= 1 && num_ray > 0.f && dim == 256, "rac_head_boundary_fwd: bad sizes B=%d Q=%d T=%d dim=%d",
+                  B, Q, T, dim);
+    if (B * Q == 0)
+        return 0;
+    RAC_CHECK_ARG(proposal && time_diff_safe && bbox_pred && bbox_xy && box_table && pc_range && pe_weight && pe_bias && pe_gamma &&
+                      pe_beta && pe_out,
+                  "rac_head_boundary_fwd: null pointer");
+    HeadBoundaryArgs a;
+    for (int i = 0; i < 2; ++i) {
+        const int rc = rg_check_desc(heads[i], i, "rac_head_boundary_fwd");
+        if (rc)
+            return rc;
+        RAC_CHECK_ARG(heads[i].num_seg == 1 && heads[i].N <= 16, "rac_head_boundary_fwd: head %d: num_seg=%d N=%d (one segment, N <= 16)", i,
+                      heads[i].num_seg, heads[i].N);
+        RAC_CHECK_ARG(!heads[i].seg[0].x_out && !heads[i].seg[0].split_out, "rac_head_boundary_fwd: head %d: no x_out / split_out", i);
+        a.d[i] = heads[i];
+    }
+    RAC_CHECK_ARG(heads[1].N == 10, "rac_head_boundary_fwd: the reg head is the 10-wide box delta (N=%d)", heads[1].N);
+    const int n = B * Q;
+    a.rows = n;
+    a.b = rac_make_boundary_args(proposal, time_diff_safe, bbox_pred, bbox_xy, box_table, pc_range, pe_weight, pe_bias, pe_gamma, pe_beta,
+                                 pe_out, Q, T, num_ray, eps);
+    hipLaunchKernelGGL(head_boundary_kernel, dim3((n + 15) / 16), dim3(256), 0, (hipStream_t)stream, a);
+    return rac_launch_status("rac_head_boundary_fwd");
+}
diff --git a/racformer_amd/fused.py b/racformer_amd/fused.py
--- a/racformer_amd/fused.py
+++ b/racformer_amd/fused.py
@@ -731,10 +731,65 @@
     return d
 
 
-def rowgemm_launch(descs, rows):
+def row_ln(a, norm, out, num_partials=1, a_scale=1.0, bias=None, residual=None):
+    j = _lib.RowLn()
+    if num_partials > 1:
+        if not a.is_contiguous() or a.shape[0] != num_partials or a.shape[-1] != 256:
+            raise RuntimeError("row_ln: partials must be a contiguous [S, rows, 256] tensor")
+        j.a, j.ld_a, j.partial_stride = ctypes.c_void_p(a.data_ptr()), 256, a.numel() // num_partials
+        keep = [a]
+    else:
+        if a.shape[-1] != 256:
+            raise RuntimeError("row_ln: rows are 256 wide")
+        t, j.a, j.ld_a = _rows2d(a, "a")
+        j.partial_stride = 0
+        keep = [t]
+    j.num_partials, j.a_scale = int(num_partials), float(a_scale)
+    if bias is not None:
+        j.bias = ctypes.c_void_p(bias.data_ptr())
+        keep.append(bias)
+    if residual is not None:
+        t, j.residual, j.ld_res = _rows2d(residual, "residual")
+        keep.append(t)
+    j.gamma, j.beta, j.eps = ctypes.c_void_p(norm.weight.data_ptr()), ctypes.c_void_p(norm.bias.data_ptr()), float(norm.eps)
+    t, j.out, j.ld_out = _rows2d(out, "out")
+    keep.append(t)
+    j._keep = keep
+    return j
+
+
+def rowgemm_launch(descs, rows, ln=None):
     arr = (_lib.RowGemm * len(descs))(*descs)
-    rc = _lib.lib().rac_rowgemm_fwd(arr, len(descs), int(rows), _lib.stream_ptr())
-    _lib.check(rc, "rac_rowgemm_fwd")
+    if ln is None:
+        rc = _lib.lib().rac_rowgemm_fwd(arr, len(descs), int(rows), _lib.stream_ptr())
+        _lib.check(rc, "rac_rowgemm_fwd")
+        return
+    rc = _lib.lib().rac_rowgemm_ln_fwd(arr, len(descs), ctypes.byref(ln), int(rows), _lib.stream_ptr())
+    _lib.check(rc, "rac_rowgemm_ln_fwd")
+
+
+def head_boundary_fused(cls_gemm, reg_gemm, proposal, time_diff_safe, num_ray, pc_range, pe_linear, pe_norm, xy_out=None):
+    proposal = proposal.contiguous()
+    _lib.require_gpu(proposal, time_diff_safe, what="head_boundary_fused")
+    B, Q, _ = proposal.shape
+    pred = torch.empty_like(proposal)
+    if xy_out is None:
+        xy = torch.empty_like(proposal)
+    else:
+        if tuple(xy_out.shape) != tuple(proposal.shape) or not xy_out.is_contiguous() or xy_out.dtype != torch.float32:
+            raise RuntimeError("head_boundary_fused: xy_out must be a contiguous float32 tensor shaped like the boxes")
+        xy = xy_out
+    table = torch.empty(B, Q, 8, device=proposal.device, dtype=torch.float32)
+    h = torch.empty(B, Q, pe_linear.weight.shape[0], device=proposal.device, dtype=torch.float32)
+    pc = (ctypes.c_float * 6)(*[float(v) for v in pc_range])
+    heads = (_lib.RowGemm * 2)(cls_gemm, reg_gemm)
+    rc = _lib.lib().rac_head_boundary_fwd(heads, _lib.ptr(proposal), _lib.ptr(time_diff_safe), _lib.ptr(pred), _lib.ptr(xy),
+                                          _lib.ptr(table), pc, _lib.ptr(pe_linear.weight), _lib.ptr(pe_linear.bias),
+                                          _lib.ptr(pe_norm.weight), _lib.ptr(pe_norm.bias), _lib.ptr(h), B, Q,
+                                          time_diff_safe.shape[1], pe_linear.weight.shape[0], float(num_ray), float(pe_norm.eps),
+                                          _lib.stream_ptr())
+    _lib.check(rc, "rac_head_boundary_fwd")
+    return pred, xy, table, h
 
 
 def pack_gemm_split_weight(weight):
diff --git a/racformer_amd/transformer.py b/racformer_amd/transformer.py
--- a/racformer_amd/transformer.py
+++ b/racformer_amd/transformer.py
@@ -10,11 +10,11 @@
 from .bbox_utils import decode_bbox, inverse_sigmoid, theta_d2xy_coods, xy2theta_d_coods
 from .fused import (SPLIT_ACT_SCALE, SPLIT_BIAS_PAD, SPLIT_SLICE, ConvImage, act_image, add_ln, bev_sampling_fused, bev_sampling_multi_fused,
                     box_prep, conv_direct, quantize_values_i16, upsample2x_image,
-                    generator_fused, gru_gate_fused, layer_boundary_fused, mixing_fused, mixing_sampled_fused, mixing_sampled_supported, outproj_fused,
+                    generator_fused, gru_gate_fused, head_boundary_fused, mixing_fused, mixing_sampled_fused, mixing_sampled_supported, outproj_fused,
                     pack_conv3x3_weight,
                     pack_gemm_split_weight,
                     pe_head, refine_fused, row_gemm,
-                    row_seg, rowgemm_launch, sampling4d_fused, sasa_fused, split_weight_f16, upsample2x_fused, value_proj_fused)
+                    row_ln, row_seg, rowgemm_launch, sampling4d_fused, sasa_fused, split_weight_f16, upsample2x_fused, value_proj_fused)
 from .msda import msda_forward
 from .msmv import msmv_forward
 
@@ -1030,12 +1030,12 @@
             sampled_feat = self._sample(qb, x1, mlvl_feats, img_metas, d_region, lin[0:3], table)
             partials = self.mixing.out_proj_partials(sampled_feat, x1, prepared["out_proj_split"], None, packs, x1_split)
         p_scale = packs["out_alpha"] if packs else 1.0
-        proj = new(2, n, E)
+        proj, x2 = new(2, n, E), new(n, E)
         ro, lo = rb.attention.output_proj, lb.attention.output_proj
         rowgemm_launch([row_gemm([row_seg(bev[0])], ro.weight, ro.bias, proj[0]),
-                        row_gemm([row_seg(bev[1])], lo.weight, lo.bias, proj[1])], n)
-        x2 = add_ln(partials, self.norm2, residual=x1, bias=self.mixing.out_proj.bias, num_partials=partials.shape[0],
-                    a_scale=p_scale)
+                        row_gemm([row_seg(bev[1])], lo.weight, lo.bias, proj[1])], n,
+                       ln=row_ln(partials, self.norm2, x2, num_partials=partials.shape[0], a_scale=p_scale,
+                                 bias=self.mixing.out_proj.bias, residual=x1))
         fk, f2k = prepared["fusion_k"], prepared["ffn2_k"]
         if len(fk) != 3 or len(f2k) != 2:
             raise RuntimeError("forward_fused: fusion must take 3 * embed_dims, feedforward_channels must be 2 * embed_dims")
@@ -1057,11 +1057,10 @@
                         row_gemm([row_seg(c0r0[:, E:])], rg[2].weight, rg[2].bias, r2, relu_from=0)], n)
         cls_score = out_slots[0] if out_slots is not None else new(B, Q, self.num_classes)
         delta = new(B, Q, self.code_size)
-        rowgemm_launch([row_gemm([row_seg(c3, norm=cb[4], relu=True)], cb[6].weight, cb[6].bias, cls_score),
-                        row_gemm([row_seg(r2)], rg[4].weight, rg[4].bias, delta)], n)
-        bbox_pred, bbox_xy, next_table, next_h = layer_boundary_fused(qb, delta, meta["time_diff_safe"], self.num_ray,
-                                                                      self.pc_range, pe[0], pe[1],
-                                                                      xy_out=out_slots[1] if out_slots is not None else None)
+        bbox_pred, bbox_xy, next_table, next_h = head_boundary_fused(
+            row_gemm([row_seg(c3, norm=cb[4], relu=True)], cb[6].weight, cb[6].bias, cls_score),
+            row_gemm([row_seg(r2)], rg[4].weight, rg[4].bias, delta), qb, meta["time_diff_safe"], self.num_ray, self.pc_range,
+            pe[0], pe[1], xy_out=out_slots[1] if out_slots is not None else None)
         self.wrote_slots = out_slots is not None
         self._carry = ((layer + 1, bbox_pred.data_ptr(), tuple(bbox_pred.shape), bbox_pred._version), next_h, next_table, bbox_pred)
         if stages is not None:
```

New measurement: 276.1, median of 6. 1.2% higher.
